# peterdavidfagan/mujoco_robot_environments

Hardware: AMD Instinct MI355X
Metric: env steps/sec (whole node), RearrangementEnv batch=4096 at 1/2/4/8 MI355X (higher is better)
Workload: dtype f32

## Files before the change

mujoco_robot_environments_amd/csrc/mre_api.cpp:

```cpp
#include <hip/hip_runtime.h>

#include <cmath>
#include <cstdio>
#include <cstdlib>
#include <cstring>
#include <string>
#include <algorithm>
#include <vector>

#include "mre_env.h"
#include "mre_labels.h"
#include "mre_heightmap.h"
#include "mre_warp.h"
#include "mre_launch.h"
#include "mre_model.h"
#include "mre_records.h"

using namespace mre;

static thread_local std::string g_err;
int mre::fail(int code, const std::string& msg) {
  g_err = msg;
  return code;
}

extern "C" const char* mre_last_error(void) { return g_err.c_str(); }

static int create_buffers(mre_env* e, int num_envs, int device_id) {
  e->N = num_envs;
  e->device = device_id;
  HIPCHK(hipSetDevice(device_id));
  HIPCHK(hipStreamCreateWithFlags(&e->stream, hipStreamNonBlocking));
  const size_t N = (size_t)num_envs;
  HIPCHK(hipMalloc(&e->dM, sizeof(DevModel)));
  HIPCHK(hipMemcpy(e->dM, &e->hM, sizeof(DevModel), hipMemcpyHostToDevice));
  HIPCHK(hipMalloc(&e->qpos, N * NQP * 4)); HIPCHK(hipMalloc(&e->qvel, N * NVP * 4));
  HIPCHK(hipMalloc(&e->qacc_ws, N * NVP * 4)); HIPCHK(hipMalloc(&e->ctrl, N * NU * 4));
  HIPCHK(hipMalloc(&e->qfine, N * QFINE_ROW * 4)); HIPCHK(hipMalloc(&e->sv_qfine, N * QFINE_ROW * 4));
  HIPCHK(hipMemsetAsync(e->qfine, 0, N * QFINE_ROW * 4, e->stream));
  HIPCHK(hipMalloc(&e->nstep, N * 4)); HIPCHK(hipMalloc(&e->sv_nstep, N * 4));
  HIPCHK(hipMemsetAsync(e->nstep, 0, N * 4, e->stream));
  HIPCHK(hipMalloc(&e->nprops, N * 4)); HIPCHK(hipMalloc(&e->prop_size, N * NPROP * 3 * 4));
  HIPCHK(hipMalloc(&e->osc_target, N * 16 * 4)); HIPCHK(hipMalloc(&e->grip_closed, N));
  HIPCHK(hipMalloc(&e->converged, N)); HIPCHK(hipMalloc(&e->mask, N));
  HIPCHK(hipMalloc(&e->sites, N * 16 * 4));
  HIPCHK(hipMalloc(&e->status, N * 4)); HIPCHK(hipMalloc(&e->stats, N * 4 * 4));
  HIPCHK(hipMalloc(&e->order, N * 4)); HIPCHK(hipMalloc(&e->auto_order, N * 4));
  HIPCHK(hipHostMalloc((void**)&e->h_auto_order, N * 4, hipHostMallocDefault));
  HIPCHK(hipStreamCreateWithFlags(&e->stream2, hipStreamNonBlocking));
  HIPCHK(hipEventCreateWithFlags(&e->ev_fork, hipEventDisableTiming));
  HIPCHK(hipEventCreateWithFlags(&e->ev_join, hipEventDisableTiming));
  HIPCHK(hipMalloc(&e->d_large, N)); HIPCHK(hipMalloc(&e->mask_r, N));
  HIPCHK(hipMalloc(&e->sv_qpos, N * NQP * 4)); HIPCHK(hipMalloc(&e->sv_qvel, N * NVP * 4));
  HIPCHK(hipMalloc(&e->sv_qacc_ws, N * NVP * 4)); HIPCHK(hipMalloc(&e->sv_ctrl, N * NU * 4));
  HIPCHK(hipMalloc(&e->sv_status, N * 4));
  HIPCHK(hipMalloc(&e->sv_converged, N));
  HIPCHK(hipHostMalloc((void**)&e->h_launch_info, mre_env::RING * N * 16, hipHostMallocMapped | hipHostMallocCoherent));
  HIPCHK(hipHostGetDevicePointer((void**)&e->d_launch_info, e->h_launch_info, 0));
  memset(e->h_launch_info, 0xFF, mre_env::RING * N * 16);
  HIPCHK(hipHostMalloc((void**)&e->h_info_last, N * 16, hipHostMallocDefault));
  memset(e->h_info_last, 0xFF, N * 16);
  HIPCHK(hipHostMalloc((void**)&e->h_large_stage, mre_env::NSTAGE * N, hipHostMallocMapped | hipHostMallocCoherent));
  HIPCHK(hipHostGetDevicePointer((void**)&e->d_large_stage, e->h_large_stage, 0));
  memset(e->h_large_stage, 0, mre_env::NSTAGE * N);
  HIPCHK(hipMalloc(&e->d_pending, N));
  HIPCHK(hipMemsetAsync(e->d_pending, 0, N, e->stream));
  HIPCHK(hipMemsetAsync(e->d_large, 0, N, e->stream));
  e->h_large.assign(N, 0); e->h_rerun.assign(N, 0);
  { int rc = sched_create(e); if (rc) return rc; }
  if (const char* fb = getenv("MRE_NO_FALLBACK")) e->fallback = atoi(fb) == 0;
  if (const char* ng = getenv("MRE_NARROW_GENERIC")) e->base_flags = atoi(ng) != 0 ? F_CLIP_ALWAYS : 0u;
  if (const char* fl = getenv("MRE_FORCE_LARGE")) {
    if (atoi(fl) != 0) {
      e->h_large.assign(N, 1); e->n_large = num_envs;
      HIPCHK(hipMemsetAsync(e->d_large, 1, N, e->stream));
    }
  }
  HIPCHK(hipMemsetAsync(e->status, 0, N * 4, e->stream)); HIPCHK(hipMemsetAsync(e->stats, 0, N * 16, e->stream));
  HIPCHK(hipMemsetAsync(e->grip_closed, 0, N, e->stream)); HIPCHK(hipMemsetAsync(e->osc_target, 0, N * 64, e->stream));
  HIPCHK(hipMemsetAsync(e->sites, 0, N * 64, e->stream));
  std::vector<int> np(N, NPROP);
  std::vector<float> ps(N * NPROP * 3, 0.0155f);
  HIPCHK(hipMemcpy(e->nprops, np.data(), N * 4, hipMemcpyHostToDevice));
  HIPCHK(hipMemcpy(e->prop_size, ps.data(), ps.size() * 4, hipMemcpyHostToDevice));
  e->osc = OscConfig{350.f, 20.f, 500.f, 100.f, 200.f, 30.f, {0.f, -0.785f, 0.f, -2.356f, 0.f, 1.571f, 0.785f},
                     5e-3f, 68e-3f, 0};
  HIPCHK(hipMalloc(&e->d_osc, sizeof(OscConfig)));
  HIPCHK(hipMemcpy(e->d_osc, &e->osc, sizeof(OscConfig), hipMemcpyHostToDevice));
  HIPCHK(hipStreamSynchronize(e->stream));
  int rc = mre_reset(e, nullptr);
  if (rc != MRE_OK) return rc;
  return mre_sync(e);
}

extern "C" int mre_create(const void* blob, size_t nbytes, int num_envs, int device_id, mre_env** out) {
  if (!blob || !out || num_envs <= 0) return fail(MRE_ERR_ARG, "mre_create: bad argument");
  *out = nullptr;
  mre_env* e = new mre_env();
  const std::string err = build_model(blob, nbytes, e->hM, e->solver);
  if (!err.empty()) { delete e; return fail(MRE_ERR_MODEL, err); }
  if (const char* it = getenv("MRE_DEBUG_ITERS")) e->hM.opt_rec.iterations = atoi(it);
  int rc;
  int ndev = 0;
  if (hipGetDeviceCount(&ndev) != hipSuccess || ndev <= 0) {
    delete e;
    return fail(MRE_ERR_NOGPU, "mre_create: no HIP device visible (the HIP path has no CPU fallback)");
  }
  if (device_id < 0 || device_id >= ndev) {
    delete e;
    return fail(MRE_ERR_ARG, "mre_create: device_id out of range");
  }
  rc = create_buffers(e, num_envs, device_id);
  if (rc != MRE_OK) {
    const std::string msg = g_err;
    mre_destroy(e);
    g_err = msg;
    return rc;
  }
  *out = e;
  return MRE_OK;
}

extern "C" int mre_destroy(mre_env* e) {
  if (!e) return MRE_OK;
  (void)hipSetDevice(e->device);
  (void)drain(e);
  if (getenv("MRE_DEBUG_TIMING") && e->dbg_calls > 0)
    fprintf(stderr, "mre: %ld pipelined calls, %.1f us per call in the library, of which %.1f us waiting for launch info\n",
            e->dbg_calls, 1e6 * e->dbg_call_s / e->dbg_calls, 1e6 * e->dbg_wait_s / e->dbg_calls);
  sched_destroy(e);
  for (float* p : e->seq_copy) if (p) (void)hipFree(p);
  if (e->stream) (void)hipStreamSynchronize(e->stream);
  if (e->stream2) (void)hipStreamSynchronize(e->stream2);
  void* ptrs[] = {e->dM, e->qpos, e->qvel, e->qacc_ws, e->ctrl, e->nprops, e->prop_size, e->osc_target,
                  e->grip_closed, e->converged, e->mask, e->sites, e->status, e->stats, e->d_osc, e->d_osc_env, e->order,
                  e->geoms, e->prop_rgb, e->bg_depth, e->bg_rgb, e->bg_seg,
                  e->d_large, e->mask_r, e->qfine, e->sv_qfine, e->nstep, e->sv_nstep, e->sv_qpos, e->sv_qvel, e->sv_qacc_ws, e->sv_ctrl,
                  e->sv_status, e->auto_order, e->sv_converged, e->contacts, e->contacts_full, e->settle_steps,
                  e->d_env_ids, e->ps_attempts, e->ps_prop, e->ps_tick, e->ps_which, e->ps_bounds, e->ps_pose, e->ps_zones,
                  e->ps_pick};
  for (void* p : ptrs) if (p) (void)hipFree(p);
  if (e->h_launch_info) (void)hipHostFree(e->h_launch_info);
  if (e->h_info_last) (void)hipHostFree(e->h_info_last);
  if (e->h_large_stage) (void)hipHostFree(e->h_large_stage);
  if (e->d_pending) (void)hipFree(e->d_pending);
  if (e->h_auto_order) (void)hipHostFree(e->h_auto_order);
  for (auto& pr : e->events) { (void)hipEventDestroy(pr.first); (void)hipEventDestroy(pr.second); }
  if (e->ev_order) (void)hipEventDestroy(e->ev_order);
  if (e->ev_fork) (void)hipEventDestroy(e->ev_fork);
  if (e->ev_join) (void)hipEventDestroy(e->ev_join);
  if (e->stream2) (void)hipStreamDestroy(e->stream2);
  if (e->stream) (void)hipStreamDestroy(e->stream);
  delete e;
  return MRE_OK;
}

extern "C" int mre_num_envs(const mre_env* e) { return e ? e->N : 0; }
extern "C" void* mre_stream(mre_env* e) { return e ? (void*)e->stream : nullptr; }
extern "C" int mre_sync(mre_env* e) {
  if (!e) return fail(MRE_ERR_ARG, "null handle");
  HIPCHK(hipSetDevice(e->device));
  DRAIN(e);
  HIPCHK(hipStreamSynchronize(e->stream));
  return MRE_OK;
}

static int copy_in(mre_env* e, void* dst, const void* src, size_t n) {
  HIPCHK(hipSetDevice(e->device));
  HIPCHK(hipMemcpyAsync(dst, src, n, hipMemcpyDefault, e->stream));
  return MRE_OK;
}
static int copy_out(mre_env* e, void* dst, const void* src, size_t n) {
  HIPCHK(hipSetDevice(e->device));
  HIPCHK(hipMemcpyAsync(dst, src, n, hipMemcpyDefault, e->stream));
  HIPCHK(hipStreamSynchronize(e->stream));
  return MRE_OK;
}
static int stage_mask(mre_env* e, const uint8_t* mask, const uint8_t** dmask) {
  *dmask = nullptr;
  if (!mask) return MRE_OK;
  int rc = copy_in(e, e->mask, mask, (size_t)e->N);
  *dmask = e->mask;
  return rc;
}

extern "C" int mre_set_props(mre_env* e, const int32_t* nprops, const float* prop_half_size) {
  if (!e || !nprops || !prop_half_size) return fail(MRE_ERR_ARG, "mre_set_props: null");
  DRAIN(e);
  int rc = copy_in(e, e->nprops, nprops, (size_t)e->N * 4);
  if (rc) return rc;
  return copy_in(e, e->prop_size, prop_half_size, (size_t)e->N * NPROP * 3 * 4);
}

extern "C" int mre_reset(mre_env* e, const uint8_t* mask) {
  if (!e) return fail(MRE_ERR_ARG, "null handle");
  DRAIN(e);
  HIPCHK(hipSetDevice(e->device));
  const uint8_t* dmask;
  int rc = stage_mask(e, mask, &dmask);
  if (rc) return rc;
  mre_launch_reset(e->dM, e->N, e->qpos, e->qvel, e->qacc_ws, e->qfine, e->ctrl, e->status, e->nstep, dmask, e->stream);
  HIPCHK(hipGetLastError());
  if (!mask) e->tick_tail_valid = false;
  bool changed = false;
  std::vector<uint8_t> hmask;
  if (mask) {
    hmask.resize((size_t)e->N);
    rc = copy_out(e, hmask.data(), dmask, (size_t)e->N);
    if (rc) return rc;
  }
  for (int i = 0; i < e->N; i++)
    if (!e->large_only && e->h_large[i] && (!mask || hmask[i])) { e->h_large[i] = 0; e->n_large--; changed = true; }
  if (changed) {
    HIPCHK(hipMemcpyAsync(e->d_large, e->h_large.data(), (size_t)e->N, hipMemcpyHostToDevice, e->stream));
    HIPCHK(hipStreamSynchronize(e->stream));
  }
  return MRE_OK;
}

static void fill_args(mre_env* e, StepArgs& a);
static bool is_device_ptr(const void* p) {
  hipPointerAttribute_t at;
  if (hipPointerGetAttributes(&at, p) != hipSuccess) { (void)hipGetLastError(); return false; }
  return at.type == hipMemoryTypeDevice;
// ... 1127 lines not shown
```

mujoco_robot_environments_amd/csrc/mre_dev.h:

```cpp
#pragma once
#include <stdint.h>

namespace mre {

constexpr int NB = 20;
constexpr int NRB = 16;
constexpr int GRIP_BODY0 = 8;
constexpr int NV = 39;
constexpr int NRV = 15;
constexpr int NQ = 43;
constexpr int NQP = 44;
constexpr int TRACE_W = 88;
constexpr int TRACE_QVEL = 48;
constexpr int NVP = 40;
constexpr int NU = 8;
constexpr int QFINE = 32;
constexpr int QFINE_ROW = 96;
constexpr int QFINE_CUBE_Q = 32;
constexpr int QFINE_CUBE_V = 60;
static_assert(QFINE_CUBE_Q + 7 * 4 == QFINE_CUBE_V && QFINE_CUBE_V + 6 * 4 <= QFINE_ROW, "qfine row layout");
constexpr int NPROP = 4;
constexpr int NG = 20;
constexpr int PROP_GEOM0 = 12;
constexpr int NPAIR = 128;
constexpr int NMR = 96;
constexpr int NSITE = 2;
constexpr int NEQ = 3;
constexpr int CONTACT_EXPORT = 32;
constexpr int MAXCHAIN = 9;
constexpr int ROBOT_DOF_PARENT[NRV] = {-1, 0, 1, 2, 3, 4, 5, 6, 7, 6, 9, 6, 11, 6, 13};
constexpr int robot_dof_depth(int i) { return ROBOT_DOF_PARENT[i] < 0 ? 0 : 1 + robot_dof_depth(ROBOT_DOF_PARENT[i]); }
constexpr int robot_dof_madr(int i) { return i == 0 ? 0 : robot_dof_madr(i - 1) + robot_dof_depth(i - 1) + 1; }
constexpr int robot_dof_anc(int i, int k) {
  int j = ROBOT_DOF_PARENT[i];
  for (int t = 0; t < k && j >= 0; t++) j = ROBOT_DOF_PARENT[j];
  return j;
}
static_assert(robot_dof_madr(NRV) == NMR, "robot mass-matrix size");

#if defined(MRE_LARGE_CAPS) && defined(MRE_NEWTON)
constexpr int NCON_MAX = 48;
constexpr int NEFC_MAX = 160;
constexpr int NRROW_MAX = 100;
constexpr int NPP_MAX = 16;
constexpr int MAXBLK = 58;
#elif defined(MRE_LARGE_CAPS)
constexpr int NCON_MAX = 44;
constexpr int NEFC_MAX = 148;
constexpr int NRROW_MAX = 83;
constexpr int NPP_MAX = 16;
constexpr int MAXBLK = 52;
#elif defined(MRE_NEWTON)
constexpr int NCON_MAX = 32;
constexpr int NEFC_MAX = 112;
constexpr int NRROW_MAX = 69;
constexpr int NPP_MAX = 8;
constexpr int MAXBLK = 40;
#else
constexpr int NCON_MAX = 32;
constexpr int NEFC_MAX = 112;
constexpr int NRROW_MAX = 62;
constexpr int NPP_MAX = 8;
constexpr int MAXBLK = 40;
#endif
constexpr int NRROW_MAX_COMPACT_PGS = 62, NRROW_MAX_COMPACT_NEWTON = 69;
#if !defined(MRE_LARGE_CAPS)
static_assert(NRROW_MAX ==
#ifdef MRE_NEWTON
              NRROW_MAX_COMPACT_NEWTON,
#else
              NRROW_MAX_COMPACT_PGS,
#endif
              "host-side copy of the compact robot-row capacity");
#endif
static_assert(NEFC_MAX <= 256 && NRROW_MAX < 127 && NPP_MAX <= 16 && MAXBLK >= 8 + NCON_MAX,
              "capacities must fit the block descriptor fields (mre_solver.h)");

struct alignas(16) PairRec {
  int g1, g2, b1, b2;
  int pid1, pid2, type1, single;
  float pos1[3], rb1;
  float pos2[3], rb2;
  float quat1[4], quat2[4];
  float size1[3], margin;
  float size2[3], gap;
};
static_assert(sizeof(PairRec) == 128, "PairRec is eight 16-byte words");

struct alignas(16) BodyRec {
  float quat[4];
  float pos[3], mass;
  float jnt_pos[3], qpos0;
  float jnt_axis[3]; int qposadr;
  float ipos[3]; int propid;
  float iquat[4];
  float inertia[3]; int dofadr;
  float jnt_range[2], invweight0[2];
  float jnt_stiffness, jnt_springref; int parent, jnt_limited;
};
static_assert(sizeof(BodyRec) == 144, "BodyRec is nine 16-byte words");
struct alignas(16) DofRec {
  int body, propid, dofadr, ten;
  float armature, damping, invweight0, ten_coef;
  float jnt_stiffness, jnt_springref, act_gain, act_bias0;
  float act_bias1, act_bias2, act_ctrl_lo, act_ctrl_hi;
  float act_force_lo, act_force_hi; int act_forcelimited, pad;
};
static_assert(sizeof(DofRec) == 80, "DofRec is five 16-byte words");
struct alignas(16) MEntryRec {
  int i, j; float armature, damping;
  float act_bias2, ten_coef; int ten, pad;
};
static_assert(sizeof(MEntryRec) == 32, "MEntryRec is two 16-byte words");
struct alignas(16) RowRec {
  float solref[2], margin, gap;
  float solimp[5], friction;
  float invw1, invw2;
};
static_assert(sizeof(RowRec) == 48, "RowRec is three 16-byte words");
constexpr int ROWREC_JNT = NEQ, ROWREC_PAIR = NEQ + NB, NROWREC = NEQ + NB + NPAIR;
struct alignas(16) EqRec {
  int type, b1, b2, pb1;
  int pb2, root, pad0, pad1;
  float data[8];
  float qpos0_1, qpos0_2; int pad2, root_chain_len;
  int root_chain[12];
};
static_assert(sizeof(EqRec) == 128 && MAXCHAIN <= 12, "EqRec is eight 16-byte words");
struct alignas(16) SiteRec {
  float pos[3]; int body;
  float quat[4];
};
static_assert(sizeof(SiteRec) == 32, "SiteRec is two 16-byte words");
struct alignas(16) OptRec {
  float timestep, impratio, tolerance; int iterations;
  float gravity[3]; int cone;
  float ten_coef[2]; int ten_dof[2];
  float grip_gainprm, grip_biasprm[3];
  float grip_forcerange[2], grip_ctrlrange[2];
  float robot_mass, M0_diag_robot_sum; int tcp_site, eef_site;
  float tcp_pos[3]; int pad;
};
static_assert(sizeof(OptRec) == 112, "OptRec is seven 16-byte words");

struct DevModel {
  int body_propid[NB];
  int chain_len[NB];
  int chain_dof[NB][MAXCHAIN];
  float body_mass[NB];
  int dof_Madr[NV + 1];
  float qpos0[NQP];
  int M_i[NMR], M_j[NMR];
  int geom_type[NG], geom_body[NG], geom_propid[NG];
  float geom_size[NG][3], geom_pos[NG][3], geom_quat[NG][4], geom_rbound[NG];
  int pair_g1[NPAIR], pair_g2[NPAIR];
  float pair_margin[NPAIR];
  PairRec pair_rec[NPAIR];
  float act_ctrlrange[NU][2];
  float home_qpos[7];
  float park_pos[NPROP][3];
  BodyRec body_rec[NB];
  DofRec dof_rec[NV];
  MEntryRec m_rec[NMR];
  RowRec row_rec[NROWREC];
  EqRec eq_rec[NEQ];
  SiteRec site_rec[NSITE];
  OptRec opt_rec;
};

struct OscConfig {
  float kp_pos, kd_pos, kp_ori, kd_ori, kp_null, kd_null;
  float null_q[7];
  float pos_thresh, ori_thresh;
  int pinv_always;
};

enum StepFlags : unsigned { F_NO_CONSTRAINTS = 1u, F_FREEZE_ROBOT = 2u, F_CONV_CONTINUE = 4u, F_CONV_OPEN = 8u,
                            F_OSC_EVAL = 16u, F_DETECT = 32u, F_SETTLE_EXIT = 64u, F_DETECT_ACTIVE = 128u,
                            F_CLIP_ALWAYS = 256u };
enum CtrlMode : int { CTRL_HELD = 0, CTRL_SEQ = 1, CTRL_OSC = 2 };

struct StepArgs {
  const DevModel* M;
  int N;
  float* qpos;
  float* qvel;
  float* qacc_ws;
  float* qfine;
  float* ctrl;
  const float* ctrl_seq;
  int seq_stride;
  const int* nprops;
  const float* prop_size;
  int nsteps, control_steps, mode;
  unsigned flags;
  const OscConfig* osc;
  int osc_stride;
  const float* osc_target;
  const uint8_t* grip_closed;
  uint8_t* converged;
  float* sites;
  uint32_t* status;
  int* nstep;
  int* stats;
  float* trace;
  int trace_nenv, trace_max, trace_base;
  const uint8_t* env_mask;
  const int* env_order;
  float* geoms;
  float* contacts;
  float* contacts_full;
  int* settle_steps;
  int min_settle_steps;
  const uint8_t* large;
  int want_large;
  float *sv_qpos, *sv_qvel, *sv_qacc_ws, *sv_qfine, *sv_ctrl;
  int* sv_nstep;
  uint32_t* sv_status;
  uint8_t* sv_converged;
  int* launch_info;
  uint8_t* pending;
  int* q_head;
  int* q_tail;
  int* q_buf;
  int* q_acc;
  int* q_done;
  int* q_started;
  const int* q_gen;
  int q_gen_expect;
  int q_wait;
  int* q_err;
  int q_nticks, q_shards, q_cap, q_stride;
  int q_lshards, q_capl;
};
constexpr int QUEUE_TICKS_MAX = 256;
constexpr int QUEUE_SHARDS_MAX = 32;
constexpr int QUEUE_LSHARDS_MAX = 16;

struct SearchArgs {
  const DevModel* M;
  int N;
  float* qpos;
  const int* nprops;
  const float* prop_size;
  const uint8_t* env_mask;
  const long long* env_ids;
  long long env_id_offset;
  unsigned long long seed;
  const int* prop;
  int fixed_prop;
  const double* bounds;
  double shared_bounds[6];
  const int* tick_base;
  long long tick0;
  int max_attempts;
  int yaw_mode;
  double fixed_quat[4];
  float max_dist;
  int commit;
  float* qfine;
  double* pose;
  int* attempts;
  unsigned flags;
};

constexpr int DYN_W = 128;
constexpr int DYN_JAC = 0, DYN_MASS = 42, DYN_BIAS = 91, DYN_POS = 98, DYN_QUAT = 101, DYN_QPOS = 105, DYN_QVEL = 112,
              DYN_PAD = 119;
struct DynArgs {
  const DevModel* M;
  int N;
  const float* qpos;
  const float* qvel;
  const float* qfine;
  const int* nprops;
  const float* prop_size;
  int site;
  float* out;
};

struct SortArgs {
  const DevModel* M;
  int N;
  const float* qpos;
  const int* nprops;
  const double* zones;
  double place_z;
  int* which;
  double* pick;
  double* bounds;
};

struct RenderArgs {
  int N, height, width;
  const float* geoms;
  const int* nprops;
  const uint8_t* prop_rgb;
  float geom_rgb[NG][3];
  float cam_pos[3], cam_mat[9];
  float fy;
  float light_pos[3];
  float ambient, head_diffuse, light_diffuse;
  float checker[2][3], checker_size;
  float zfar;
  uint8_t* rgb;
  float* depth;
  uint8_t* seg;
  const uint8_t* env_mask;
  int g0, g1;
  const float* bg_depth;
  const uint8_t* bg_rgb;
  const uint8_t* bg_seg;
};

}
```

mujoco_robot_environments_amd/csrc/mre_kernels.hip:

```cpp
#include <hip/hip_runtime.h>

#include "mre_dev.h"
#include "mre_math.h"
#include "mre_collide.h"

namespace mre {
using ModelP = MRE_MODEL_PTR(DevModel);
#if defined(MRE_PHASE_STAMPS) && MRE_PHASE_STAMPS >= 4
__shared__ unsigned long long dbg_acc[4];
#endif

struct OscSm {
  float J[6][7], M[7][7], MiJt[7][6], Li[6][6], Lam[6][6], V[6][6], Jbar[7][6];
  float ep[3], eo[3], F[6], LF[6], tn[7], Jbt[6], xd[6], w[6];
};

struct alignas(8) Blk {
  uint16_t row0;
  uint8_t type, nrows;
  uint8_t rslot;
  uint8_t pa, pb;
  uint8_t primary : 4;
  uint8_t bslot : 4;
};

constexpr int TAB_BYTES = 8 * (MAXBLK * 5 + 1) + 4 * 48;
constexpr int FRAME_BYTES = (int)sizeof(OscSm) > 4 * (NB * 16) ? (int)sizeof(OscSm) : 4 * (NB * 16);
constexpr int R1_MIN = TAB_BYTES - FRAME_BYTES > 0 ? TAB_BYTES - FRAME_BYTES : 4;
constexpr int MD_LD = 17;

struct Sm {
  float qpos[NQP], qvel[NVP], qlo[QFINE], ctrl[NU];
  float qfrc_smooth[NVP], qacc_smooth[NVP], qacc[NVP], qfrc_bias[NVP], qfrc_con[NVP];
  union {
    struct { float xpos[NB][3], xquat[NB][4], xmat[NB][9]; };
    OscSm osc;
#ifdef MRE_NEWTON
    struct { float nw_Ma[NVP], nw_grad[NVP], nw_search[NVP], nw_Mv[NVP]; };
#endif
  };
#ifndef MRE_NEWTON
  char tab_room[R1_MIN];
#endif
  float cdof[NRV][6];
  union {
    struct { float con_pos[NCON_MAX][3], con_frame[NCON_MAX][9], con_dist[NCON_MAX]; };
#ifdef MRE_NEWTON
    struct { float jar[NEFC_MAX], frc[NEFC_MAX], jv[NEFC_MAX]; };
#else
    struct { float jar[NEFC_MAX], frc[NEFC_MAX], pyr_f[4 * NCON_MAX]; };
#endif
  };
  float com_robot[3];
  float site_xpos[NSITE][3], site_xmat[1][9];
#ifdef MRE_NEWTON
  float qM[NMR];
#else
  float qM[NMR], qLD[NMR], qLDinv[NRV + 1];
#endif
  float prop_mass[NPROP], prop_inertia[NPROP][3], prop_size[NPROP][3];
  union { float scratch[64]; int iscr[64]; };
  float osc_tgt[16];
  int nprops;
  int ncon, nefc, nl, nrrow, npp, overflow, solver_iters;
  int finger_contact;
  uint8_t con_pair[NCON_MAX], con_rslot[NCON_MAX], con_bslot[NCON_MAX], con_b1[NCON_MAX], con_b2[NCON_MAX];
  uint16_t lim_info[NRV + 1];
  union {
    float JpA[3 * NCON_MAX][6];
    struct {
      float cinert[NB][10], crb[NRB][10], gP[NRB - GRIP_BODY0][6], gC[NRB - GRIP_BODY0][6];
      double gpose[NRB - GRIP_BODY0][7];
    };
  };
  float JpB[3 * NPP_MAX][6];
  union {
    float Jr[NRROW_MAX][NRV];
    struct {
      float cdof_dot[NV][6], cvel[NB][6], cfrc[NB][6];
      alignas(8) double gI[NRB - GRIP_BODY0][10];
      double gS[NRB - GRIP_BODY0][6];
    };
  };
#ifdef MRE_NEWTON
  float efc_R[NEFC_MAX], efc_aref[NEFC_MAX];
  float frc_r[NRROW_MAX];
  float con_fric[NCON_MAX];
  float hc[NCON_MAX][6];
  float Md[NRV][MD_LD];
  alignas(8) float W[NV * (NV + 1) / 2];
  uint8_t rstate[NEFC_MAX];
  uint8_t clist[NPROP][NCON_MAX];
  uint8_t ccount[NPROP], cpl_robot, cpl_cubes;
  alignas(8) uint16_t jdesc[NEFC_MAX][4];
  float zrow[24];
#else
  float Br[NRROW_MAX][NRV];
  alignas(16) float blkrec[MAXBLK][16];
  Blk blk[MAXBLK];
  uint8_t sched[MAXBLK][8];
#endif
  uint16_t hdr[NEFC_MAX];

  int nblk, nsched;
};

#if defined(MRE_LARGE_CAPS)
static_assert(sizeof(Sm) <= 27136, "large-capacity Sm must fit 6 workgroups per CU");
#else
static_assert(sizeof(Sm) <= 20480, "compact Sm must fit 8 workgroups per CU");
#endif

#ifdef MRE_NEWTON
MRE_DEV float* mh_store(Sm& s) { return &s.JpA[0][0]; }
static_assert(sizeof(((Sm*)0)->JpA) >= sizeof(float) * NMR, "M - h dF/dv fits the head of the constraint block");
#else
MRE_DEV float* mh_store(Sm& s) { return s.qLD; }
#endif

struct BodyRegs {
  float anchor[3], axis[3], xipos[3], ximat[9];
};

MRE_DEV double robot_q(const Sm& s, int d) { return (double)s.qpos[d] + (double)s.qlo[d]; }
MRE_DEV double robot_v(const Sm& s, int d) { return (double)s.qvel[d] + (double)s.qlo[QFINE / 2 + d]; }

MRE_DEV bool prop_is_active(const Sm& s, int propid) { return propid < 0 || propid < s.nprops; }

struct BodyK {
  float quat[4], pos[3], mass, jnt_pos[3], qpos0, jnt_axis[3], ipos[3], iquat[4], inertia[3];
  int qposadr, propid, dofadr, parent;
};
MRE_DEV BodyK load_body(ModelP M, int b) {
  const auto* R = &M->body_rec[b];
  BodyK B;
#pragma unroll
  for (int k = 0; k < 4; k++) { B.quat[k] = R->quat[k]; B.iquat[k] = R->iquat[k]; }
#pragma unroll
  for (int k = 0; k < 3; k++) { B.pos[k] = R->pos[k]; B.jnt_pos[k] = R->jnt_pos[k]; B.jnt_axis[k] = R->jnt_axis[k];
                                B.ipos[k] = R->ipos[k]; B.inertia[k] = R->inertia[k]; }
  B.mass = R->mass; B.qpos0 = R->qpos0; B.qposadr = R->qposadr; B.propid = R->propid; B.dofadr = R->dofadr;
  B.parent = R->parent;
  return B;
}

MRE_DEV bool body_is_active(ModelP M, const Sm& s, int b) {
  int p = M->body_propid[b];
  return p < 0 || p < s.nprops;
}

MRE_DEV void sincos_poly_d(double x, double& sn, double& cs) {
  const double z = x * x;
  double ps = -1.0 / 1307674368000.0;
  ps = ps * z + 1.0 / 6227020800.0;
  ps = ps * z - 1.0 / 39916800.0;
  ps = ps * z + 1.0 / 362880.0;
// ... 1143 lines not shown
  if (QUEUE && !Q_LARGE && l == 0) __hip_atomic_fetch_add(a.q_started, 1, __ATOMIC_RELAXED, __HIP_MEMORY_SCOPE_AGENT);
  if (QUEUE && Q_LARGE && a.q_wait != 0) {
    for (unsigned idle = 0; q_load(a.q_gen) != a.q_gen_expect; ++idle) {
      if (idle > 1024u) return;
      __builtin_amdgcn_s_sleep(127);
    }
  }
 for (;;) {
  if (QUEUE) {
    if (!queue_pop(a, l, (int)(blockIdx.x % (unsigned)(Q_LARGE ? a.q_lshards : a.q_shards)), env, qtick, qshard)) return;
    if (qtick > 0 || Q_LARGE) __builtin_amdgcn_fence(__ATOMIC_ACQUIRE, "agent");
  }
  const int step_lo = QUEUE ? qtick * a.control_steps : 0, step_hi = QUEUE ? step_lo + a.control_steps : a.nsteps;
  if (QUEUE && !Q_LARGE && qtick == 0 && a.large != nullptr && a.large[env] != 0) continue;
  if (!QUEUE || (!Q_LARGE && qtick == 0)) {
#define MRE_PASS_SKIP { if (QUEUE) { if (l == 0) __hip_atomic_fetch_add(a.q_done, 1, __ATOMIC_RELAXED, __HIP_MEMORY_SCOPE_AGENT); continue; } return; }
  if (!QUEUE && a.large != nullptr && (a.large[env] != 0) != (a.want_large != 0)) return;
  if (a.env_mask != nullptr && a.env_mask[env] == 0) {
    if (a.launch_info != nullptr && l < 4) a.launch_info[(size_t)env * 4 + l] = -1;
    MRE_PASS_SKIP;
  }
  if (a.pending != nullptr && a.pending[env] != 0) {
    if (a.launch_info != nullptr && l < 4) a.launch_info[(size_t)env * 4 + l] = l == 0 ? -2 : -1;
    MRE_PASS_SKIP;
  }
#undef MRE_PASS_SKIP
  }
  ModelP M = (ModelP)a.M;

  const bool save = a.sv_qpos != nullptr && step_lo == 0;
  if (l < NQP) {
    const float v = a.qpos[(size_t)env * NQP + l];
    s.qpos[l] = v;
    if (save) a.sv_qpos[(size_t)env * NQP + l] = v;
  }
  if (l < NVP) {
    const float v = a.qvel[(size_t)env * NVP + l], w = a.qacc_ws[(size_t)env * NVP + l];
    s.qvel[l] = v;
    s.qacc[l] = w;
    s.qfrc_con[l] = 0.f;
    if (save) { a.sv_qvel[(size_t)env * NVP + l] = v; a.sv_qacc_ws[(size_t)env * NVP + l] = w; }
  }
  if (l < QFINE) {
    const float v = a.qfine != nullptr ? a.qfine[(size_t)env * QFINE_ROW + l] : 0.f;
    s.qlo[l] = v;
    if (save && a.qfine != nullptr) a.sv_qfine[(size_t)env * QFINE_ROW + l] = v;
  }
  if (save && a.qfine != nullptr && l < QFINE_ROW - QFINE)
    a.sv_qfine[(size_t)env * QFINE_ROW + QFINE + l] = a.qfine[(size_t)env * QFINE_ROW + QFINE + l];
  float cube_lo_keep = 0.f;
  if (QUEUE && !Q_LARGE && a.qfine != nullptr && l < QFINE_ROW - QFINE) cube_lo_keep = a.qfine[(size_t)env * QFINE_ROW + QFINE + l];
  if (l < NU) {
    const float v = a.ctrl[(size_t)env * NU + l];
    s.ctrl[l] = v;
    if (save) a.sv_ctrl[(size_t)env * NU + l] = v;
  }
  if (save && l == 0) {
    if (a.nstep != nullptr) a.sv_nstep[env] = a.nstep[env];
    a.sv_status[env] = a.status[env];
    a.sv_converged[env] = a.converged != nullptr ? a.converged[env] : (uint8_t)0;
  }
  if (l == 0) { s.nprops = a.nprops[env]; s.overflow = 0; s.ncon = 0; s.nefc = 0; s.solver_iters = 0; }
#ifdef MRE_NEWTON
  if (l < 24) s.zrow[l] = 0.f;
#endif
  if (l < NPROP * 3) {
    const float sz = a.prop_size[(size_t)env * NPROP * 3 + l];
    s.prop_size[l / 3][l % 3] = sz;
  }
  MRE_SYNC();
  if (l < NPROP) {
    const float m = M->body_mass[NRB + l];
    const float* z = s.prop_size[l];
    s.prop_mass[l] = m;
    s.prop_inertia[l][0] = m / 3.f * (z[1] * z[1] + z[2] * z[2]);
    s.prop_inertia[l][1] = m / 3.f * (z[0] * z[0] + z[2] * z[2]);
    s.prop_inertia[l][2] = m / 3.f * (z[0] * z[0] + z[1] * z[1]);
  }
  MRE_SYNC();

#if defined(MRE_PHASE_STAMPS) && MRE_PHASE_STAMPS >= 4
  if (l < 4) dbg_acc[l] = 0ull;
#endif
#ifdef MRE_PHASE_STAMPS
  unsigned long long stamp_acc[4] = {0, 0, 0, 0};
  unsigned long long stamp_t = __builtin_amdgcn_s_memtime();
#endif
  bool arm_converged = ((a.flags & F_CONV_CONTINUE) != 0 || (QUEUE && qtick > 0)) && a.converged != nullptr && a.converged[env] != 0;
  float grip_cmd = 0.f;
  const OscConfig* oscp = a.osc + (size_t)env * a.osc_stride;
  int hw_ncon = 0, hw_nefc = 0, hw_nrrow = 0, hw_npp = 0;
  const unsigned long long launch_t0 = __builtin_amdgcn_s_memtime();
  if (a.mode == CTRL_OSC) {
    if (l < 16) s.osc_tgt[l] = a.osc_target[(size_t)env * 16 + l];
    grip_cmd = a.grip_closed[env] ? M->act_ctrlrange[NU - 1][1] : M->act_ctrlrange[NU - 1][0];
    MRE_SYNC();
  }
  int steps_done = 0;
  bool settled = false;
  for (int step = step_lo; step < step_hi; ++step) {
    MRE_STAMP(7);
    position_stage(M, s, l);
    MRE_STAMP(12);
    MRE_STAMP(13);
    gripper_local(M, s, l);
    if ((a.flags & F_NO_CONSTRAINTS) == 0) connect_rows_local(M, s, l);
    MRE_STAMP(14);
    crb_mass_matrix(M, s, l);
    MRE_SYNC();
#ifndef MRE_NEWTON
    factor_robot_regs(s.qM, s.qLD, s.qLDinv);
#endif
    MRE_STAMP(15);
    MRE_STAMP(0);

    velocity_stage(M, s, l);
    MRE_SYNC();
    finger_bias(M, s, l);
    MRE_STAMP(1);
    const bool constrained = (a.flags & F_NO_CONSTRAINTS) == 0;
    if (constrained) {

      collide(M, s, l, false, (a.flags & F_CLIP_ALWAYS) != 0);
      MRE_STAMP(2);
      assemble_constraints(M, s, l);
#ifdef MRE_NEWTON
      nw_build_lists(s, l);
#else
      solve_robot_rows(s, l);
      assemble_blocks(M, s, l);
#endif
      MRE_STAMP(3);
      hw_ncon = max(hw_ncon, s.ncon); hw_nefc = max(hw_nefc, s.nefc);
      hw_nrrow = max(hw_nrrow, s.nrrow); hw_npp = max(hw_npp, s.npp);
    }

    if (a.mode == CTRL_SEQ && (step % a.control_steps) == 0) {
      const int tick = step / a.control_steps;
      if (l < NU) s.ctrl[l] = a.ctrl_seq[((size_t)tick * a.seq_stride + env) * NU + l];
      MRE_SYNC();
    }
    if (a.mode == CTRL_OSC && (step % a.control_steps) == 0) {
      if (step > 0 && osc_converged(M, s, oscp, s.osc_tgt)) arm_converged = true;
      osc_compute(M, s, osc, oscp, s.osc_tgt, l);
      if (l == 0) s.ctrl[NU - 1] = grip_cmd;
      MRE_SYNC();
    }
    MRE_STAMP(4);
    const unsigned clamped = smooth_forces(M, s, l);
    MRE_STAMP(5);
    bool polished = false;
    if (constrained) {
#if defined(MRE_NEWTON) && defined(MRE_PHASE_STAMPS)
      newton_solve(M, s, l, stamp_acc, stamp_t);
      polished = nw_robot_polish(M, s, l);
#elif defined(MRE_NEWTON)
      newton_solve(M, s, l);
      polished = nw_robot_polish(M, s, l);
#else
      if (M->opt_rec.cone == 0) solve_constraints_pyramidal(M, s, l);
      else solve_constraints(M, s, l);
#endif
      MRE_STAMP(6);
    } else {
      if (l < NVP) { s.qacc[l] = s.qacc_smooth[l]; s.qfrc_con[l] = 0.f; }
      MRE_SYNC();
    }

    integrate_setup(M, s, l, clamped);
    factor_solve_robot(mh_store(s), s.scratch, l);
    integrate(M, s, l, a.flags, polished, a.qfine != nullptr ? a.qfine + (size_t)env * QFINE_ROW + QFINE_CUBE_Q : nullptr);
    steps_done = step + 1 - step_lo;
    if ((a.flags & F_SETTLE_EXIT) != 0) {
      float mv = 0.f, ma = 0.f;
      if (l >= NRV && l < NRV + 6 * s.nprops) { mv = fabsf(s.qvel[l]); ma = fabsf(s.qacc[l]); }
      mv = wave_max(mv); ma = wave_max(ma);
      settled = mv < 1e-3f && ma < 1e-2f && step + 1 > a.min_settle_steps;
    }
    if (a.trace != nullptr && env < a.trace_nenv && (a.trace_base + step) < a.trace_max) {
      if (l < TRACE_QVEL) {
        float v = l < NQ ? s.qpos[l] : 0.f;
        if (l == NQ && constrained) {
          int mask = 0;
          for (int k = 0; k < s.nl; k++) mask |= 1 << ((s.lim_info[k] & 0xFF) - 1);
          v = (float)(s.ncon + 64 * mask);
        }
        if (l == NQ + 1 && constrained) {
          unsigned h = 0u;
          for (int c = 0; c < s.ncon; c++) {
            const int pr = s.con_pair[c];
            const unsigned key = (unsigned)(M->pair_g1[pr] * 32 + M->pair_g2[pr] + 1);
            h = (h + key * key) & 0x3FFFFFu;
          }
          v = (float)h;
        }
        if (l == NQ + 2 && constrained && M->opt_rec.cone != 0) {
          unsigned h = 0u;
          const int ns = 7 + s.nl;
          for (int i = 7; i < ns; i++) h += (s.frc[i] > 0.f ? 1u : 2u) * (unsigned)((i + 1) * (i + 1));
          for (int c = 0; c < s.ncon; c++) {
            const int i = ns + 3 * c;
#ifdef MRE_NEWTON
            const float mu = s.con_fric[c];
#else
            const float mu = s.blkrec[8 + c][15];
#endif
            const float fn = s.frc[i], ft2 = s.frc[i + 1] * s.frc[i + 1] + s.frc[i + 2] * s.frc[i + 2], lim = mu * fn;
            const unsigned z = fn <= 0.f ? 1u : (ft2 >= lim * lim * (1.f - 1e-4f) ? 3u : 2u);
            h += z * (unsigned)((c + 3) * (c + 3));
          }
          v = (float)(h & 0x3FFFFFu);
        }
        a.trace[((size_t)(a.trace_base + step) * a.trace_nenv + env) * TRACE_W + l] = v;
      }
      if (l < NVP) a.trace[((size_t)(a.trace_base + step) * a.trace_nenv + env) * TRACE_W + TRACE_QVEL + l] = l < NV ? s.qvel[l] : 0.f;
    }
    if (settled) break;
  }
  MRE_STAMP(7);
  if (a.settle_steps != nullptr && l == 0) a.settle_steps[env] = settled ? steps_done : -steps_done;
  const bool hand_over = QUEUE && !Q_LARGE && s.overflow != 0;
  if (a.nstep != nullptr && l == 0 && !hand_over) {
    if (QUEUE) __hip_atomic_fetch_add(a.nstep + env, steps_done, __ATOMIC_RELAXED, __HIP_MEMORY_SCOPE_AGENT);
    else a.nstep[env] += steps_done;
  }
  if (a.nsteps == 0 && (a.flags & F_OSC_EVAL) != 0 && a.mode == CTRL_OSC) {
    position_stage(M, s, l);
    gripper_local(M, s, l);
    crb_mass_matrix(M, s, l);
    MRE_SYNC();
    velocity_stage(M, s, l);
    MRE_SYNC();
    osc_compute(M, s, osc, oscp, s.osc_tgt, l);
    if (l == 0) s.ctrl[NU - 1] = grip_cmd;
    MRE_SYNC();
  }
  if (a.nsteps == 0 && (a.flags & F_DETECT) != 0 && a.contacts != nullptr) {
    position_stage(M, s, l);
    collide(M, s, l, (a.flags & F_DETECT_ACTIVE) == 0, (a.flags & F_CLIP_ALWAYS) != 0);
    float* o = a.contacts + (size_t)env * (1 + 3 * CONTACT_EXPORT);
    const int n = s.ncon < CONTACT_EXPORT ? s.ncon : CONTACT_EXPORT;
    if (l == 0) o[0] = s.overflow ? -(float)s.ncon : (float)s.ncon;
    if (l < n) {
      const int pr = s.con_pair[l];
      o[1 + 3 * l] = (float)M->pair_g1[pr]; o[2 + 3 * l] = (float)M->pair_g2[pr]; o[3 + 3 * l] = s.con_dist[l];
      if (a.contacts_full != nullptr) {
        float* f = a.contacts_full + ((size_t)env * CONTACT_EXPORT + l) * 12;
        for (int k = 0; k < 3; k++) f[k] = s.con_pos[l][k];
        for (int k = 0; k < 9; k++) f[3 + k] = s.con_frame[l][k];
      }
    }
    MRE_SYNC();
    if (l == 0) s.overflow = 0;
  }
  const bool q_last = !QUEUE || (qtick + 1 == a.q_nticks && !hand_over);
  if (q_last && (a.mode == CTRL_OSC || a.sites != nullptr || a.geoms != nullptr)) kinematics_only(M, s, l);
  if (a.mode == CTRL_OSC && a.nsteps > 0 && !hand_over) {
    if (q_last && osc_converged(M, s, oscp, s.osc_tgt)) arm_converged = true;
    if (l == 0) {
      if (a.converged != nullptr) a.converged[env] = arm_converged ? 1 : 0;
      if (q_last && !arm_converged && a.status != nullptr && (a.flags & F_CONV_OPEN) == 0) {
        if (QUEUE) __hip_atomic_fetch_or(a.status + env, 1u, __ATOMIC_RELAXED, __HIP_MEMORY_SCOPE_AGENT);
        else a.status[env] |= 1u;
      }
    }
  }
  if (a.geoms != nullptr && l < NG) {
    float p[3], R[9], size[3], rb;
    geom_pose(M, s, l, p, R, size, &rb);
    float* o = a.geoms + ((size_t)env * NG + l) * 16;
    const int pid = M->geom_propid[l];
    const bool active = pid < 0 || pid < s.nprops;
    for (int k = 0; k < 3; k++) o[k] = p[k];
    for (int k = 0; k < 9; k++) o[3 + k] = R[k];
    for (int k = 0; k < 3; k++) o[12 + k] = size[k];
    o[15] = active ? (float)M->geom_type[l] : -1.f;
  }
  if (a.sites != nullptr && q_last) {
    float* o = a.sites + (size_t)env * 16;
    if (l < 3) o[l] = s.site_xpos[M->opt_rec.tcp_site][l];
    if (l >= 3 && l < 6) o[l] = s.site_xpos[M->opt_rec.eef_site][l - 3];
    if (l == 6) {
      float q[4];
      mat2q(q, s.site_xmat[0]);
      o[6] = q[0]; o[7] = q[1]; o[8] = q[2]; o[9] = q[3];
    }
  }
  if (hand_over) {
    if (a.qfine != nullptr && l < QFINE_ROW - QFINE) a.qfine[(size_t)env * QFINE_ROW + QFINE + l] = cube_lo_keep;
  } else {
    if (l < NQP) a.qpos[(size_t)env * NQP + l] = s.qpos[l];
    if (l < NVP) {
      a.qvel[(size_t)env * NVP + l] = s.qvel[l];
      a.qacc_ws[(size_t)env * NVP + l] = l < NV ? s.qacc[l] : 0.f;
    }
    if (l < QFINE && a.qfine != nullptr) a.qfine[(size_t)env * QFINE_ROW + l] = s.qlo[l];
    if (l < NU) a.ctrl[(size_t)env * NU + l] = s.ctrl[l];
  }
  const bool q_more = QUEUE && !hand_over && qtick + 1 < a.q_nticks;
  if (l == 0 && a.launch_info != nullptr) {
    int* li = a.launch_info + (size_t)env * 4;
    unsigned long long dt = (__builtin_amdgcn_s_memtime() - launch_t0) >> 10;
    int moved = 0;
    if (QUEUE) {
      int* qa = a.q_acc + (size_t)env * 4;
      if (qtick > 0 || Q_LARGE) {
        hw_ncon = max(hw_ncon, q_load(qa + 0) & 0xFFFF); hw_nefc = max(hw_nefc, q_load(qa + 1));
        hw_nrrow = max(hw_nrrow, q_load(qa + 2) & 0xFFFF); hw_npp = max(hw_npp, q_load(qa + 2) >> 16);
        dt += (unsigned long long)q_load(qa + 3);
        moved = q_load(qa + 0) >> 16;
// ... 437 lines not shown
```

mujoco_robot_environments_amd/csrc/mre_model.cpp:

```cpp
#include "mre_model.h"

#include <cstdint>
#include <cstring>
#include <vector>

#include "../../include/mre.h"

namespace mre {

namespace {
struct Blob {
  const unsigned char* p;
  size_t n;
  bool find(const char* name, uint32_t* code, uint32_t* count, uint64_t* off) const {
    uint32_t ne;
    memcpy(&ne, p + 8, 4);
    const unsigned char* t = p + 16;
    for (uint32_t k = 0; k < ne; k++, t += 48)
      if (strncmp((const char*)t, name, 32) == 0) {
        memcpy(code, t + 32, 4); memcpy(count, t + 36, 4); memcpy(off, t + 40, 8);
        return *off + (size_t)(*count) * (*code ? 8 : 4) <= n;
      }
    return false;
  }
  bool ints(const char* name, int* dst, int expect) const {
    uint32_t c, cnt; uint64_t off;
    if (!find(name, &c, &cnt, &off) || c != 0 || (int)cnt != expect) return false;
    memcpy(dst, p + off, 4 * (size_t)cnt);
    return true;
  }
  bool flts(const char* name, float* dst, int expect) const {
    uint32_t c, cnt; uint64_t off;
    if (!find(name, &c, &cnt, &off) || c != 1 || (int)cnt != expect) return false;
    for (uint32_t k = 0; k < cnt; k++) {
      double v;
      memcpy(&v, p + off + 8 * (size_t)k, 8);
      dst[k] = (float)v;
    }
    return true;
  }
};
}

#define RI(name, dst, n) if (!b.ints(name, (int*)(dst), n)) return std::string("model entry ") + name
#define RF(name, dst, n) if (!b.flts(name, (float*)(dst), n)) return std::string("model entry ") + name

static bool same_bits(const void* a, const void* b, size_t n) { return memcmp(a, b, n) == 0; }
static std::string pack_records(const ModelTables& t, DevModel& m) {
  if (t.ten_dof[0] == t.ten_dof[1] || t.ten_dof[0] < 0 || t.ten_dof[0] >= NRV || t.ten_dof[1] < 0 || t.ten_dof[1] >= NRV)
    return "the gripper tendon must couple two different robot dofs";
  for (int e = 0; e < NEQ; e++)
    for (int k = 0; k < 2; k++)
      if (t.eq_obj[e][k] < 1 || t.eq_obj[e][k] >= NRB) return "equality constraints must couple robot bodies";
  if (t.tcp_site < 0 || t.tcp_site >= NSITE || t.eef_site < 0 || t.eef_site >= NSITE) return "tcp_site / eef_site name no site";
  for (int b = 1; b < NRB; b++)
    if (t.body_parent[b] != ROBOT_DOF_PARENT[b - 1] + 1) return "robot body tree differs from the one the kernels are unrolled for (mre_dev.h)";
  for (int d = 0; d < NV; d++)
    if (t.dof_body[d] != (d < NRV ? d + 1 : NRB + (d - NRV) / 6)) return "dof layout differs from the compiled kernels";
  auto ten_of = [&](int d) { return d == t.ten_dof[0] ? 0 : (d == t.ten_dof[1] ? 1 : -1); };
  for (int b = 0; b < NB; b++) {
    BodyRec& r = m.body_rec[b];
    memset(&r, 0, sizeof(r));
    for (int c = 0; c < 4; c++) { r.quat[c] = t.body_quat[b][c]; r.iquat[c] = t.body_iquat[b][c]; }
    for (int c = 0; c < 3; c++) { r.pos[c] = t.body_pos[b][c]; r.ipos[c] = t.body_ipos[b][c]; r.jnt_pos[c] = t.jnt_pos[b][c];
                                  r.jnt_axis[c] = t.jnt_axis[b][c]; r.inertia[c] = t.body_inertia[b][c]; }
    for (int c = 0; c < 2; c++) { r.jnt_range[c] = t.jnt_range[b][c]; r.invweight0[c] = t.body_invweight0[b][c]; }
    r.mass = t.body_mass[b]; r.qposadr = t.body_qposadr[b]; r.dofadr = t.body_dofadr[b]; r.propid = t.body_propid[b];
    r.qpos0 = (r.qposadr >= 0 && r.qposadr < NQ) ? t.qpos0[r.qposadr] : 0.f;
    r.jnt_stiffness = t.jnt_stiffness[b]; r.jnt_springref = t.jnt_springref[b];
    r.parent = t.body_parent[b]; r.jnt_limited = t.jnt_limited[b];
  }
  for (int d = 0; d < NV; d++) {
    DofRec& r = m.dof_rec[d];
    memset(&r, 0, sizeof(r));
    const int b = t.dof_body[d];
    if (b < 0 || b >= NB) return "dof_bodyid names a body that does not exist";
    r.body = b; r.propid = t.body_propid[b]; r.dofadr = t.body_dofadr[b]; r.ten = ten_of(d);
    r.armature = t.dof_armature[d]; r.damping = t.dof_damping[d]; r.invweight0 = t.dof_invweight0[d];
    r.ten_coef = r.ten >= 0 ? t.ten_coef[r.ten] : 0.f;
    r.jnt_stiffness = t.jnt_stiffness[b]; r.jnt_springref = t.jnt_springref[b];
    if (d < 7) {
      r.act_gain = t.act_gain[d]; r.act_bias0 = t.act_bias[d][0]; r.act_bias1 = t.act_bias[d][1]; r.act_bias2 = t.act_bias[d][2];
      r.act_ctrl_lo = t.act_ctrlrange[d][0]; r.act_ctrl_hi = t.act_ctrlrange[d][1];
      r.act_force_lo = t.act_forcerange[d][0]; r.act_force_hi = t.act_forcerange[d][1];
      r.act_forcelimited = t.act_forcelimited[d];
    }
  }
  for (int e = 0; e < NMR; e++) {
    MEntryRec& r = m.m_rec[e];
    memset(&r, 0, sizeof(r));
    r.i = t.M_i[e]; r.j = t.M_j[e];
    r.armature = t.dof_armature[r.i]; r.damping = t.dof_damping[r.i];
    r.act_bias2 = r.i < 7 ? t.act_bias[r.i][2] : 0.f;
    r.ten = ten_of(r.i); r.ten_coef = r.ten >= 0 ? t.ten_coef[r.ten] : 0.f;
  }
  for (int k = 0; k < NROWREC; k++) memset(&m.row_rec[k], 0, sizeof(RowRec));
  for (int e = 0; e < NEQ; e++) {
    RowRec& r = m.row_rec[e];
    const int b1 = t.eq_obj[e][0], b2 = t.eq_obj[e][1];
    for (int c = 0; c < 2; c++) r.solref[c] = t.eq_solref[e][c];
    for (int c = 0; c < 5; c++) r.solimp[c] = t.eq_solimp[e][c];
    r.invw1 = e < 2 ? t.body_invweight0[b1][0] : t.dof_invweight0[b1 - 1];
    r.invw2 = e < 2 ? t.body_invweight0[b2][0] : t.dof_invweight0[b2 - 1];
    EqRec& q = m.eq_rec[e];
    memset(&q, 0, sizeof(q));
    q.type = t.eq_type[e]; q.b1 = b1; q.b2 = b2; q.pb1 = t.body_parent[b1]; q.pb2 = t.body_parent[b2];
    q.root = b1;
    while (q.root >= GRIP_BODY0) q.root = t.body_parent[q.root];
    for (int c = 0; c < 8; c++) q.data[c] = t.eq_data[e][c];
    q.qpos0_1 = t.qpos0[b1 - 1]; q.qpos0_2 = t.qpos0[b2 - 1];
    q.root_chain_len = t.chain_len[q.root];
    for (int c = 0; c < MAXCHAIN; c++) q.root_chain[c] = t.chain_dof[q.root][c];
  }
  for (int b = 1; b < NRB; b++) {
    RowRec& r = m.row_rec[ROWREC_JNT + b];
    for (int c = 0; c < 2; c++) r.solref[c] = t.jnt_solref[b][c];
    for (int c = 0; c < 5; c++) r.solimp[c] = t.jnt_solimp[b][c];
    r.invw1 = t.dof_invweight0[b - 1];
  }
  for (int k = 0; k < NPAIR; k++) {
    if (t.pair_g1[k] < 0) continue;
    RowRec& r = m.row_rec[ROWREC_PAIR + k];
    const int b1 = t.geom_body[t.pair_g1[k]], b2 = t.geom_body[t.pair_g2[k]];
    for (int c = 0; c < 2; c++) r.solref[c] = t.pair_solref[k][c];
    for (int c = 0; c < 5; c++) r.solimp[c] = t.pair_solimp[k][c];
    r.margin = t.pair_margin[k]; r.gap = t.pair_gap[k]; r.friction = t.pair_friction[k][0];
    r.invw1 = (b1 > 0 && b1 < NRB) ? t.body_invweight0[b1][0] : 0.f;
    r.invw2 = (b2 > 0 && b2 < NRB) ? t.body_invweight0[b2][0] : 0.f;
  }
  for (int k = 0; k < NSITE; k++) {
    SiteRec& r = m.site_rec[k];
    memset(&r, 0, sizeof(r));
    if (t.site_body[k] < 0 || t.site_body[k] >= NB) return "site_bodyid names a body that does not exist";
    r.body = t.site_body[k];
    for (int c = 0; c < 3; c++) r.pos[c] = t.site_pos[k][c];
    for (int c = 0; c < 4; c++) r.quat[c] = t.site_quat[k][c];
  }
  {
    OptRec& o = m.opt_rec;
    memset(&o, 0, sizeof(o));
    o.timestep = t.timestep; o.impratio = t.impratio; o.tolerance = t.tolerance; o.iterations = t.iterations;
    for (int c = 0; c < 3; c++) { o.gravity[c] = t.gravity[c]; o.grip_biasprm[c] = t.grip_biasprm[c]; }
    o.cone = t.cone;
    for (int c = 0; c < 2; c++) { o.ten_coef[c] = t.ten_coef[c]; o.ten_dof[c] = t.ten_dof[c]; o.grip_forcerange[c] = t.grip_forcerange[c];
                                  o.grip_ctrlrange[c] = t.act_ctrlrange[NU - 1][c]; }
    o.grip_gainprm = t.grip_gainprm; o.robot_mass = t.robot_mass; o.M0_diag_robot_sum = t.M0_diag_robot_sum;
    o.tcp_site = t.tcp_site; o.eef_site = t.eef_site;
    for (int c = 0; c < 3; c++) o.tcp_pos[c] = t.site_pos[t.tcp_site][c];
  }

  bool ok = true;
#define SAME(a, b) ok = ok && sizeof(a) == sizeof(b) && same_bits(&(a), &(b), sizeof(a))
  for (int b = 0; b < NB && ok; b++) {
    const BodyRec& r = m.body_rec[b];
    SAME(r.quat, t.body_quat[b]); SAME(r.pos, t.body_pos[b]); SAME(r.mass, t.body_mass[b]); SAME(r.jnt_pos, t.jnt_pos[b]);
    SAME(r.jnt_axis, t.jnt_axis[b]); SAME(r.qposadr, t.body_qposadr[b]); SAME(r.ipos, t.body_ipos[b]);
    SAME(r.propid, t.body_propid[b]); SAME(r.iquat, t.body_iquat[b]); SAME(r.inertia, t.body_inertia[b]);
    SAME(r.dofadr, t.body_dofadr[b]); SAME(r.jnt_range, t.jnt_range[b]); SAME(r.invweight0, t.body_invweight0[b]);
    SAME(r.jnt_stiffness, t.jnt_stiffness[b]); SAME(r.jnt_springref, t.jnt_springref[b]); SAME(r.parent, t.body_parent[b]);
    SAME(r.jnt_limited, t.jnt_limited[b]);
    if (b >= 1) SAME(r.qpos0, t.qpos0[t.body_qposadr[b]]);
  }
  for (int d = 0; d < NV && ok; d++) {
    const DofRec& r = m.dof_rec[d];
    const int b = t.dof_body[d];
    SAME(r.body, t.dof_body[d]); SAME(r.propid, t.body_propid[b]); SAME(r.dofadr, t.body_dofadr[b]);
    ok = ok && r.ten == (d == t.ten_dof[0] ? 0 : (d == t.ten_dof[1] ? 1 : -1));
    SAME(r.armature, t.dof_armature[d]); SAME(r.damping, t.dof_damping[d]); SAME(r.invweight0, t.dof_invweight0[d]);
    if (r.ten >= 0) SAME(r.ten_coef, t.ten_coef[r.ten]);
    SAME(r.jnt_stiffness, t.jnt_stiffness[b]); SAME(r.jnt_springref, t.jnt_springref[b]);
    if (d < 7) {
      SAME(r.act_gain, t.act_gain[d]); SAME(r.act_bias0, t.act_bias[d][0]); SAME(r.act_bias1, t.act_bias[d][1]);
      SAME(r.act_bias2, t.act_bias[d][2]); SAME(r.act_ctrl_lo, t.act_ctrlrange[d][0]); SAME(r.act_ctrl_hi, t.act_ctrlrange[d][1]);
      SAME(r.act_force_lo, t.act_forcerange[d][0]); SAME(r.act_force_hi, t.act_forcerange[d][1]);
      SAME(r.act_forcelimited, t.act_forcelimited[d]);
    }
  }
  for (int e = 0; e < NMR && ok; e++) {
    const MEntryRec& r = m.m_rec[e];
    SAME(r.i, t.M_i[e]); SAME(r.j, t.M_j[e]);
    const int i = t.M_i[e];
    SAME(r.armature, t.dof_armature[i]); SAME(r.damping, t.dof_damping[i]);
    if (i < 7) SAME(r.act_bias2, t.act_bias[i][2]);
    ok = ok && r.ten == (i == t.ten_dof[0] ? 0 : (i == t.ten_dof[1] ? 1 : -1));
    if (r.ten >= 0) SAME(r.ten_coef, t.ten_coef[r.ten]);
  }
  for (int e = 0; e < NEQ && ok; e++) {
    const RowRec& r = m.row_rec[e];
    const EqRec& q = m.eq_rec[e];
    const int b1 = t.eq_obj[e][0], b2 = t.eq_obj[e][1];
    SAME(r.solref, t.eq_solref[e]); SAME(r.solimp, t.eq_solimp[e]);
    if (e < 2) { SAME(r.invw1, t.body_invweight0[b1][0]); SAME(r.invw2, t.body_invweight0[b2][0]); }
    else { SAME(r.invw1, t.dof_invweight0[b1 - 1]); SAME(r.invw2, t.dof_invweight0[b2 - 1]); }
    SAME(q.type, t.eq_type[e]); SAME(q.b1, t.eq_obj[e][0]); SAME(q.b2, t.eq_obj[e][1]);
    SAME(q.pb1, t.body_parent[b1]); SAME(q.pb2, t.body_parent[b2]); SAME(q.data, t.eq_data[e]);
    SAME(q.qpos0_1, t.qpos0[b1 - 1]); SAME(q.qpos0_2, t.qpos0[b2 - 1]);
    int root = b1;
    while (root >= GRIP_BODY0) root = t.body_parent[root];
    ok = ok && q.root == root;
    SAME(q.root_chain_len, t.chain_len[root]);
    for (int c = 0; c < MAXCHAIN; c++) SAME(q.root_chain[c], t.chain_dof[root][c]);
  }
  for (int b = 1; b < NRB && ok; b++) {
    const RowRec& r = m.row_rec[ROWREC_JNT + b];
    SAME(r.solref, t.jnt_solref[b]); SAME(r.solimp, t.jnt_solimp[b]); SAME(r.invw1, t.dof_invweight0[b - 1]);
  }
  for (int k = 0; k < NPAIR && ok; k++) {
    if (t.pair_g1[k] < 0) continue;
    const RowRec& r = m.row_rec[ROWREC_PAIR + k];
    const int b1 = t.geom_body[t.pair_g1[k]], b2 = t.geom_body[t.pair_g2[k]];
    SAME(r.solref, t.pair_solref[k]); SAME(r.solimp, t.pair_solimp[k]); SAME(r.margin, t.pair_margin[k]);
    SAME(r.gap, t.pair_gap[k]); SAME(r.friction, t.pair_friction[k][0]);
    if (b1 > 0 && b1 < NRB) SAME(r.invw1, t.body_invweight0[b1][0]);
    if (b2 > 0 && b2 < NRB) SAME(r.invw2, t.body_invweight0[b2][0]);
  }
  for (int k = 0; k < NSITE && ok; k++) {
    const SiteRec& r = m.site_rec[k];
    SAME(r.body, t.site_body[k]); SAME(r.pos, t.site_pos[k]); SAME(r.quat, t.site_quat[k]);
  }
  {
    const OptRec& o = m.opt_rec;
    SAME(o.timestep, t.timestep); SAME(o.impratio, t.impratio); SAME(o.tolerance, t.tolerance); SAME(o.iterations, t.iterations);
    SAME(o.gravity, t.gravity); SAME(o.cone, t.cone); SAME(o.ten_coef, t.ten_coef); SAME(o.ten_dof, t.ten_dof);
    SAME(o.grip_gainprm, t.grip_gainprm); SAME(o.grip_biasprm, t.grip_biasprm); SAME(o.grip_forcerange, t.grip_forcerange);
    SAME(o.grip_ctrlrange, t.act_ctrlrange[NU - 1]); SAME(o.robot_mass, t.robot_mass);
    SAME(o.M0_diag_robot_sum, t.M0_diag_robot_sum); SAME(o.tcp_site, t.tcp_site); SAME(o.eef_site, t.eef_site);
    SAME(o.tcp_pos, t.site_pos[t.tcp_site]);
  }
#undef SAME
  if (!ok) return "a packed model record differs from the table it was filled from";
  return std::string();
}

std::string build_model(const void* blob, size_t nbytes, DevModel& m, int& solver) {
  if (nbytes < 16) return "blob too small";
  Blob b{(const unsigned char*)blob, nbytes};
  uint32_t magic;
  memcpy(&magic, b.p, 4);
  if (magic != 0x4D524542u) return "bad blob magic";
  uint32_t nentry;
  memcpy(&nentry, b.p + 8, 4);
  if (16 + 48 * (size_t)nentry > nbytes) return "blob too small";
  ModelTables t;
  memset(&t, 0, sizeof(t));
  memset(&m, 0, sizeof(m));
  int nbody, nv, nq, nM, ngeom, nsite, npair, neq, nprop, nu;
  RI("nbody", &nbody, 1); RI("nv", &nv, 1); RI("nq", &nq, 1); RI("nM", &nM, 1); RI("ngeom", &ngeom, 1);
  RI("nsite", &nsite, 1); RI("npair", &npair, 1); RI("neq", &neq, 1); RI("nprop", &nprop, 1);
  RI("nu", &nu, 1);
  if (nbody != NB || nv != NV || nq != NQ || ngeom != NG || nsite != NSITE || npair > NPAIR ||
      neq != NEQ || nprop != NPROP || nu != NU)
    return "scene dimensions differ from the compiled kernels";
  int body_jnttype[NB], act_dof[NU];
  RI("body_parentid", t.body_parent, NB); RI("body_jnttype", body_jnttype, NB);
  RI("body_dofadr", t.body_dofadr, NB); RI("body_qposadr", t.body_qposadr, NB);
  RI("body_propid", t.body_propid, NB);
  RF("body_pos", t.body_pos, NB * 3); RF("body_quat", t.body_quat, NB * 4);
  RF("body_ipos", t.body_ipos, NB * 3); RF("body_iquat", t.body_iquat, NB * 4);
  RF("body_mass", t.body_mass, NB); RF("body_inertia", t.body_inertia, NB * 3);
  RF("body_invweight0", t.body_invweight0, NB * 2);
  RF("jnt_pos", t.jnt_pos, NB * 3); RF("jnt_axis", t.jnt_axis, NB * 3); RF("jnt_range", t.jnt_range, NB * 2);
  RF("jnt_stiffness", t.jnt_stiffness, NB); RF("jnt_springref", t.jnt_springref, NB);
  RF("jnt_solref", t.jnt_solref, NB * 2); RF("jnt_solimp", t.jnt_solimp, NB * 5);
  RI("jnt_limited", t.jnt_limited, NB);
  RI("dof_bodyid", t.dof_body, NV); RI("dof_parentid", t.dof_parent, NV); RI("dof_Madr", t.dof_Madr, NV);
  t.dof_Madr[NV] = nM;
  RF("dof_armature", t.dof_armature, NV); RF("dof_damping", t.dof_damping, NV);
  RF("dof_invweight0", t.dof_invweight0, NV); RF("qpos0", t.qpos0, NQ);
  RI("geom_type", t.geom_type, NG); RI("geom_bodyid", t.geom_body, NG); RI("geom_propid", t.geom_propid, NG);
  RF("geom_size", t.geom_size, NG * 3); RF("geom_pos", t.geom_pos, NG * 3);
  RF("geom_quat", t.geom_quat, NG * 4); RF("geom_rbound", t.geom_rbound, NG);
  {
    std::vector<int> pg(2 * npair);
    RI("pair_geom", pg.data(), 2 * npair);
    for (int k = 0; k < NPAIR; k++) { t.pair_g1[k] = -1; t.pair_g2[k] = -1; }
    for (int k = 0; k < npair; k++) { t.pair_g1[k] = pg[2 * k]; t.pair_g2[k] = pg[2 * k + 1]; }
  }
  RI("pair_single", t.pair_single, npair);
  RF("pair_friction", t.pair_friction, npair * 3); RF("pair_solref", t.pair_solref, npair * 2);
  RF("pair_solimp", t.pair_solimp, npair * 5); RF("pair_margin", t.pair_margin, npair);
  RF("pair_gap", t.pair_gap, npair);
  for (int k = 0; k < NPAIR; k++) {
    PairRec& r = m.pair_rec[k];
    memset(&r, 0, sizeof(r));
    r.g1 = t.pair_g1[k]; r.g2 = t.pair_g2[k];
    if (r.g1 < 0) { r.g2 = -1; r.b1 = r.b2 = 0; r.pid1 = r.pid2 = -1; continue; }
    if (r.g1 >= NG || r.g2 < 0 || r.g2 >= NG) return "pair table names a geom that does not exist";
    r.b1 = t.geom_body[r.g1]; r.b2 = t.geom_body[r.g2];
    r.pid1 = t.geom_propid[r.g1]; r.pid2 = t.geom_propid[r.g2];
    r.type1 = t.geom_type[r.g1]; r.single = (t.pair_single[k] & 0xFF) | (t.geom_type[r.g2] << 8);
    if (t.geom_type[r.g1] == 2 || (t.geom_type[r.g2] == 2 && t.geom_type[r.g1] != 1))
      return "cylinder pairs: only box (geom 1) - cylinder (geom 2) is implemented";
    for (int c = 0; c < 3; c++) { r.pos1[c] = t.geom_pos[r.g1][c]; r.pos2[c] = t.geom_pos[r.g2][c];
                                  r.size1[c] = t.geom_size[r.g1][c]; r.size2[c] = t.geom_size[r.g2][c]; }
    for (int c = 0; c < 4; c++) { r.quat1[c] = t.geom_quat[r.g1][c]; r.quat2[c] = t.geom_quat[r.g2][c]; }
    r.rb1 = t.geom_rbound[r.g1]; r.rb2 = t.geom_rbound[r.g2];
    r.margin = t.pair_margin[k]; r.gap = t.pair_gap[k];
  }
  RI("site_bodyid", t.site_body, NSITE); RF("site_pos", t.site_pos, NSITE * 3);
  RF("site_quat", t.site_quat, NSITE * 4);
  RI("eef_site", &t.eef_site, 1); RI("tcp_site", &t.tcp_site, 1);
  RI("eq_type", t.eq_type, NEQ); RI("eq_obj", t.eq_obj, NEQ * 2); RF("eq_data", t.eq_data, NEQ * 8);
  RF("eq_solref", t.eq_solref, NEQ * 2); RF("eq_solimp", t.eq_solimp, NEQ * 5);
  RI("ten_dof", t.ten_dof, 2); RF("ten_coef", t.ten_coef, 2);
  RI("act_dof", act_dof, NU); RF("act_ctrlrange", t.act_ctrlrange, NU * 2);
  RF("grip_gainprm", &t.grip_gainprm, 1); RF("grip_biasprm", t.grip_biasprm, 3);
  RF("grip_forcerange", t.grip_forcerange, 2);
  for (int a = 0; a < NU; a++) { t.act_gain[a] = 1.f; t.act_forcelimited[a] = 0; }
  { uint32_t c, cnt; uint64_t off;
    if (b.find("act_gainprm", &c, &cnt, &off)) {
      RF("act_gainprm", t.act_gain, NU); RF("act_biasprm", t.act_bias, NU * 3);
      RF("act_forcerange", t.act_forcerange, NU * 2); RI("act_forcelimited", t.act_forcelimited, NU);
    } }
  RF("opt_timestep", &t.timestep, 1); RF("opt_gravity", t.gravity, 3); RF("opt_impratio", &t.impratio, 1);
  RF("opt_tolerance", &t.tolerance, 1); RI("opt_iterations", &t.iterations, 1);
  solver = MRE_SOLVER_PGS;
  { uint32_t c, cnt; uint64_t off; if (b.find("opt_solver", &c, &cnt, &off)) RI("opt_solver", &solver, 1); }
  if (solver != MRE_SOLVER_PGS && solver != MRE_SOLVER_NEWTON) return "opt_solver must be 0 (PGS) or 2 (Newton)";
  { uint32_t c, cnt; uint64_t off; int cone = 1;
    if (b.find("opt_cone", &c, &cnt, &off)) RI("opt_cone", &cone, 1);
    if (cone != 0 && cone != 1) return "opt_cone must be 0 (pyramidal) or 1 (elliptic)";
    t.cone = cone; }
  RF("home_qpos", t.home_qpos, 7);
  float M0d[NV];
  RF("M0_diag", M0d, NV);

  for (int bb = 1; bb < NB; bb++) {
    bool ok = bb < NRB ? (body_jnttype[bb] == 1 && t.body_dofadr[bb] == bb - 1 && t.body_qposadr[bb] == bb - 1 &&
                          t.body_propid[bb] < 0 && t.body_parent[bb] < bb)
                       : (body_jnttype[bb] == 2 && t.body_dofadr[bb] == NRV + 6 * (bb - NRB) &&
                          t.body_qposadr[bb] == NRV + 7 * (bb - NRB) && t.body_propid[bb] == bb - NRB &&
                          t.body_parent[bb] == 0);
    if (!ok) return "body layout differs from the compiled kernels";
  }
  if (t.dof_Madr[NRV] != NMR) return "robot mass-matrix size differs";
  for (int a = 0; a < 7; a++)
    if (act_dof[a] != a) return "arm actuators must drive dofs 0..6";

  int body_level[NB] = {0};
  for (int bb = 1; bb < NB; bb++) body_level[bb] = body_level[t.body_parent[bb]] + 1;
  for (int bb = 0; bb < NB; bb++)
    if (body_level[bb] > MAXCHAIN) return "tree deeper than MAXCHAIN";

  t.robot_mass = 0;
  for (int bb = 1; bb < NRB; bb++) {
    t.robot_mass += t.body_mass[bb];
    int chain[MAXCHAIN], n = 0;
    for (int d = t.body_dofadr[bb]; d >= 0; d = t.dof_parent[d]) {
      if (n >= MAXCHAIN) return "dof chain too long";
      chain[n++] = d;
    }
    t.chain_len[bb] = n;
    for (int k = 0; k < n; k++) t.chain_dof[bb][k] = chain[n - 1 - k];
  }
  for (int i = 0; i < NRV; i++) {
    int adr = t.dof_Madr[i];
    for (int j = i; j >= 0; j = t.dof_parent[j], adr++) { t.M_i[adr] = i; t.M_j[adr] = j; }
    if (adr != t.dof_Madr[i + 1]) return "dof_Madr inconsistent";
  }
  for (int i = 0; i < NRV; i++)
    if (t.dof_parent[i] != ROBOT_DOF_PARENT[i] || t.dof_Madr[i] != robot_dof_madr(i))
      return "robot dof tree differs from the one the kernels are unrolled for (mre_dev.h)";
  t.M0_diag_robot_sum = 0;
  for (int i = 0; i < NRV; i++) t.M0_diag_robot_sum += M0d[i];
  for (int p = 0; p < NPROP; p++) {
    t.park_pos[p][0] = 2.0f + 0.5f * p; t.park_pos[p][1] = 2.0f; t.park_pos[p][2] = -5.0f;
  }
#define KEEP(x) static_assert(sizeof(m.x) == sizeof(t.x), #x); memcpy(&m.x, &t.x, sizeof(m.x))
  KEEP(body_propid); KEEP(chain_len); KEEP(chain_dof); KEEP(body_mass);
  KEEP(dof_Madr); KEEP(qpos0); KEEP(M_i); KEEP(M_j);
  KEEP(geom_type); KEEP(geom_body); KEEP(geom_propid); KEEP(geom_size); KEEP(geom_pos); KEEP(geom_quat); KEEP(geom_rbound);
  KEEP(pair_g1); KEEP(pair_g2); KEEP(pair_margin);
  KEEP(act_ctrlrange); KEEP(home_qpos); KEEP(park_pos);
#undef KEEP
  std::string err = pack_records(t, m);
  if (!err.empty()) return err;
  int prop_geom0 = -1;
  for (int g = 0; g < NG; g++) if (t.geom_propid[g] == 0) prop_geom0 = g;
  if (prop_geom0 != PROP_GEOM0 || t.geom_type[1] != 1 || t.geom_body[1] != 0)
    return "mre_create: expected geom 1 = the table (static box) and one geom per cube slot";
  return std::string();
}

}
```

mujoco_robot_environments_amd/csrc/mre_newton.h:

```cpp
#pragma once

namespace mre {

constexpr int NW_QUAD = 0, NW_SAT = 1, NW_CONE = 4;
constexpr int NW_LS_MAX = 20;
constexpr float NW_LS_TOL = 0.01f;
#ifndef NW_LS_REL_VALUE
#define NW_LS_REL_VALUE 1e-5f
#endif
constexpr float NW_LS_REL = NW_LS_REL_VALUE;

MRE_DEV float rdlane(float v, int lane) {
  return __builtin_bit_cast(float, __builtin_amdgcn_readlane(__builtin_bit_cast(int, v), lane));
}
MRE_DEV int uni(int v) { return __builtin_amdgcn_readfirstlane(v); }
MRE_DEV float unif(float v) {
  return __builtin_bit_cast(float, __builtin_amdgcn_readfirstlane(__builtin_bit_cast(int, v)));
}

MRE_DEV float nw_Jl(const Sm& s, int i, int h, int l, int lp, int lk) {
  const int rs = h & 0xFF, pa = (h >> 8) & 0xF, pb = (h >> 12) & 0xF;
  float j = 0.f;
  if (l < NRV) {
    if (rs != HDR_NONE) j = s.Jr[rs][l];
// ... 162 lines not shown
#pragma unroll
      for (int q = 0; q < 8; q++)
        if (g0 + q < n) t[q] = rdlane(u, HI - g0 - q);
      __builtin_amdgcn_sched_barrier(0);
#pragma unroll
      for (int q = 0; q < 8; q++)
        if (g0 + q < n) hh[HI - g0 - q] = fmaf(-u, t[q], hh[HI - g0 - q]);
      __builtin_amdgcn_sched_barrier(0);
    }
  }
}

template <int K>
MRE_DEV void nw_elim_col(float (&hh)[NV], float& g, float& y, float& dinv, int l, unsigned nbm) {
  constexpr int blk = K < NRV ? 0 : 1 + (K - NRV) / 6;
  constexpr int b0 = blk == 0 ? 0 : NRV + 6 * (blk - 1);
  const float piv = rdlane(hh[K], K);
  const float d = __builtin_amdgcn_rsqf(fmaxf(piv, 1e-20f));
  const float u = hh[K] * d;
  hh[K] = u;
  const float yk = rdlane(g, K) * d;
  g = fmaf(-u, yk, g);
  y = (l == K) ? yk : y;
  dinv = (l == K) ? d : dinv;
  nw_elim_update<K - 1, b0>(hh, u);
  if constexpr (blk > 0) {
    if constexpr (blk > 3) { if (nbm & (1u << 3)) nw_elim_update<NRV + 17, NRV + 12>(hh, u); }
    if constexpr (blk > 2) { if (nbm & (1u << 2)) nw_elim_update<NRV + 11, NRV + 6>(hh, u); }
    if constexpr (blk > 1) { if (nbm & (1u << 1)) nw_elim_update<NRV + 5, NRV>(hh, u); }
    if (nbm & 1u) nw_elim_update<NRV - 1, 0>(hh, u);
  }
}
template <int K, int KEND>
MRE_DEV void nw_elim_range(float (&hh)[NV], float& g, float& y, float& dinv, int l, unsigned nbm) {
  nw_elim_col<K>(hh, g, y, dinv, l, nbm);
  if constexpr (K > KEND) nw_elim_range<K - 1, KEND>(hh, g, y, dinv, l, nbm);
}

struct NwPoint { float alpha, cost, d1, d2; };

MRE_PHASE_FN void nw_build_lists(Sm& s, int l) {
  const int kept = s.ncon;
  const bool on = l < kept;
  const int cb1 = on ? s.con_b1[l] : 0, cb2 = on ? s.con_b2[l] : 0;
  int pa = -1, pb = -1;
  if (cb1 >= NRB) pa = cb1 - NRB;
  if (cb2 >= NRB) { if (pa < 0) pa = cb2 - NRB; else pb = cb2 - NRB; }
  const unsigned long long lt = (1ull << l) - 1ull;
  const bool rob = on && pa >= 0 && s.con_rslot[on ? l : 0] != HDR_NONE;
  unsigned cr = 0u, cc = 0u;
#pragma unroll
  for (int p = 0; p < NPROP; p++) {
    const bool mine = on && (pa == p || pb == p);
    const unsigned long long m = __ballot(mine);
    if (mine) s.clist[p][__popcll(m & lt)] = (uint8_t)(pb == p ? (l | 0x80) : l);
    if (l == 0) s.ccount[p] = (uint8_t)__popcll(m);
    if (__ballot(rob && pa == p) != 0ull) cr |= 1u << p;
  }
  const int pairbit = (on && pb >= 0) ? cube_pair_bit(pa, pb) : -1;
#pragma unroll
  for (int b = 0; b < 6; b++)
    if (__ballot(pairbit == b) != 0ull) cc |= 1u << b;
  if (l == 0) { s.cpl_robot = (uint8_t)cr; s.cpl_cubes = (uint8_t)cc; }
  const int nscalar = 7 + s.nl;
  const unsigned zoff = (unsigned)offsetof(Sm, zrow);
  for (int i = l; i < s.nefc; i += 64) {
    const int h = s.hdr[i], ra = (h >> 8) & 0xF, rb = (h >> 12) & 0xF;
    const int crow = i - nscalar;
    const unsigned offA = crow >= 0 ? (unsigned)offsetof(Sm, JpA) + 24u * (unsigned)crow : zoff;
    const unsigned offB = (crow >= 0 && rb != 0xF)
                              ? (unsigned)offsetof(Sm, JpB) + 24u * (unsigned)(3 * s.con_bslot[crow / 3] + crow % 3) : zoff;
#pragma unroll
    for (int cb = 0; cb < NPROP; cb++) s.jdesc[i][cb] = (uint16_t)(ra == cb ? offA : (rb == cb ? offB : zoff));
  }
  MRE_SYNC();
}

struct NwLane {
  int lp, lk;
  bool lact;
  float mdiag;
  float mu_scale;
  float scale;
};
MRE_DEV NwLane nw_lane(ModelP M, const Sm& s, int l) {
  NwLane c;
  c.lp = (l >= NRV && l < NV) ? (l - NRV) / 6 : -1;
  c.lk = (l >= NRV && l < NV) ? (l - NRV) % 6 : 0;
  c.lact = l < NRV || (c.lp >= 0 && c.lp < s.nprops);
  c.mdiag = c.lp >= 0 ? (c.lk < 3 ? s.prop_mass[c.lp] : s.prop_inertia[c.lp][c.lk - 3]) : 0.f;
  c.mu_scale = __builtin_amdgcn_rsqf(fmaxf(M->opt_rec.impratio, kMinVal));
  float msum = M->opt_rec.M0_diag_robot_sum;
  for (int p = 0; p < s.nprops; p++)
    msum += 3.f * s.prop_mass[p] + s.prop_inertia[p][0] + s.prop_inertia[p][1] + s.prop_inertia[p][2];
  c.scale = 1.0f / msum;
  return c;
}

template <bool PYR>
MRE_DEV float nw_update_gradient(Sm& s, int l, const NwLane& c, int nscalar, int ncon) {
  const float sc = nw_update<true, PYR>(s, l, nscalar, ncon, c.mu_scale, s.jar);
  MRE_SYNC();
  const float qc = nw_JTf(s, l, c.lp, c.lk, nscalar);
  const bool on = l < NV && c.lact;
  const float fs = on ? s.qfrc_smooth[l] : 0.f, as = on ? s.qacc_smooth[l] : 0.f;
  const float qa = on ? s.qacc[l] : 0.f, Ma = on ? s.nw_Ma[l] : 0.f;
  if (l < NVP) {
    s.qfrc_con[l] = on ? qc : 0.f;
    s.nw_grad[l] = on ? Ma - fs - qc : 0.f;
  }
  const float cost = sc + wave_sum(0.5f * (Ma - fs) * (qa - as));
  MRE_SYNC();
  return cost;
}

template <bool PYR>
MRE_DEV float nw_setup_impl(ModelP M, Sm& s, int l) {
  const NwLane c = nw_lane(M, s, l);
  const int nefc = s.nefc, ncon = s.ncon, nscalar = 7 + s.nl;
  for (int e = l; e < NRV * MD_LD; e += 64) (&s.Md[0][0])[e] = 0.f;
  MRE_SYNC();
  for (int e = l; e < NMR; e += 64) {
    const int i = M->M_i[e], j = M->M_j[e];
    const float v = s.qM[e];
    s.Md[i][j] = v; s.Md[j][i] = v;
  }
  MRE_SYNC();
  const bool on = l < NV && c.lact;
  const float fs = on ? s.qfrc_smooth[l] : 0.f, as = on ? s.qacc_smooth[l] : 0.f;
  float qa = on ? s.qacc[l] : 0.f;
  float Ma = on ? nw_mulM(s, l, c.mdiag, s.qacc) : 0.f;
  for (int i = l; i < nefc; i += 64) {
    const float aref = s.efc_aref[i];
    float d1, d2;
    row_dot2(s, i, s.qacc, s.qacc_smooth, d1, d2);
    s.jar[i] = d1 - aref;
    s.jv[i] = d2 - aref;
  }
  MRE_SYNC();
  const float gauss = wave_sum(0.5f * (Ma - fs) * (qa - as));
  const float cost_ws = gauss + nw_update<false, PYR>(s, l, nscalar, ncon, c.mu_scale, s.jar);
  const float cost_sm = nw_update<false, PYR>(s, l, nscalar, ncon, c.mu_scale, s.jv);
  if (cost_ws > cost_sm || !(cost_ws == cost_ws)) {
    qa = as; Ma = fs;
    for (int i = l; i < nefc; i += 64) s.jar[i] = s.jv[i];
  }
  if (l < NVP) { s.qacc[l] = qa; s.nw_Ma[l] = Ma; }
  MRE_SYNC();
  return nw_update_gradient<PYR>(s, l, c, nscalar, ncon);
}
MRE_PHASE_FN float nw_setup(ModelP M, Sm& s, int l) { return nw_setup_impl<false>(M, s, l); }
MRE_PHASE_FN float nw_setup_pyramidal(ModelP M, Sm& s, int l) { return nw_setup_impl<true>(M, s, l); }

MRE_PHASE_FN void nw_direction(ModelP M, Sm& s, int l) {
  MRE_DBG_T0();
  const NwLane c = nw_lane(M, s, l);
  const int nefc = s.nefc, nscalar = 7 + s.nl, nprops = s.nprops;
  const int lp = c.lp, lk = c.lk;
  float hh[NV];
#pragma unroll
  for (int k = 0; k < NV; k++) {
    float v = 0.f;
    if (k < NRV) { if (l < NRV) v = s.Md[l][k]; }
    else if (l == k) v = c.lact ? c.mdiag : 1.0f;
    hh[k] = v;
  }
  MRE_DBG_STAMP(4, 0);
#if defined(MRE_PHASE_STAMPS) && MRE_PHASE_STAMPS == 5
  {
    int nc_ = 0, nq_ = 0;
    for (int r0 = 0; r0 < nefc; r0 += 64) {
      const int st_ = r0 + l < nefc ? (int)s.rstate[r0 + l] : NW_SAT;
      nc_ += __popcll(__ballot(st_ == NW_CONE)); nq_ += __popcll(__ballot(st_ == NW_QUAD));
    }
    if (threadIdx.x == 0) { dbg_acc[2] += (unsigned long long)nc_ << 4; dbg_acc[3] += (unsigned long long)nq_ << 4; }
  }
#endif
  typedef float v4f __attribute__((ext_vector_type(4)));
  v4f c00 = {0.f, 0.f, 0.f, 0.f}, c10 = c00, c11 = c00, c20 = c00, c21 = c00, c22 = c00;
  {
    const int g = l >> 4, m16 = l & 15;
    const char* const sb = reinterpret_cast<const char*>(&s);
    const unsigned zoff = (unsigned)offsetof(Sm, zrow), jr0 = (unsigned)offsetof(Sm, Jr);
    const unsigned sh = m16 < 12 ? 16u * (unsigned)(m16 / 6) : 0u;
    const unsigned lo = 4u * (unsigned)(m16 % 6), lr = 4u * (unsigned)m16;
    auto ldw = [&](unsigned off) { return *reinterpret_cast<const float*>(sb + off); };
    auto meta = [&](int r0, int& ii, int& st, int& h, float& R, uint2& d) {
      const int i = r0 + g;
      ii = i < nefc ? i : 0;
      st = i < nefc ? (int)s.rstate[ii] : NW_SAT;
      h = s.hdr[ii];
      R = s.efc_R[ii];
      d = *reinterpret_cast<const uint2*>(&s.jdesc[ii][0]);
    };
    auto gather = [&](int h, uint2 d, float& w0, float& w1, float& w2) {
      const int rs = h & 0xFF;
      w0 = ldw((rs != HDR_NONE ? jr0 + 60u * (unsigned)rs : zoff) + lr);
      w1 = ldw(((d.x >> sh) & 0xFFFFu) + lo);
      w2 = nprops > 2 ? ldw(((d.y >> sh) & 0xFFFFu) + lo) : 0.f;
    };
    static_assert(sizeof(s.Jr[0]) == 60 && sizeof(s.JpA[0]) == 24 && sizeof(s.JpB[0]) == 24, "row strides of the gathers");
    struct Meta { int ii, st, h; float R; uint2 d; };
    auto chunk = [&](const Meta& cur, Meta& nxt, int r0) {
      const int ii = cur.ii, h = cur.h, st = cur.st;
      const uint2 d = cur.d;
      const bool quad = st == NW_QUAD, cone = st == NW_CONE;
      const float D = quad ? __builtin_amdgcn_rcpf(cur.R) : 0.f;
      if (r0 + 4 < nefc) meta(r0 + 4, nxt.ii, nxt.st, nxt.h, nxt.R, nxt.d);
      float v0, v1, v2, a0, a1, a2;
      if (__any(cone)) {
        const int cr = ii - nscalar;
        const int k = cone ? cr % 3 : 0;
        const int i0 = ii - k, i1 = cone ? i0 + 1 : ii, i2 = cone ? i0 + 2 : ii;
        float x0, x1, x2, y0, y1, y2, z0, z1, z2;
        gather(s.hdr[i0], *reinterpret_cast<const uint2*>(&s.jdesc[i0][0]), x0, x1, x2);
        gather(s.hdr[i1], *reinterpret_cast<const uint2*>(&s.jdesc[i1][0]), y0, y1, y2);
        gather(s.hdr[i2], *reinterpret_cast<const uint2*>(&s.jdesc[i2][0]), z0, z1, z2);
        const float* hcp = s.hc[cone ? cr / 3 : 0];
        const float H0 = k == 0 ? hcp[0] : (k == 1 ? hcp[1] : hcp[2]);
        const float H1 = k == 0 ? hcp[1] : (k == 1 ? hcp[3] : hcp[4]);
        const float H2 = k == 0 ? hcp[2] : (k == 1 ? hcp[4] : hcp[5]);
        v0 = k == 0 ? x0 : (k == 1 ? y0 : z0);
        v1 = k == 0 ? x1 : (k == 1 ? y1 : z1);
        v2 = k == 0 ? x2 : (k == 1 ? y2 : z2);
        a0 = cone ? H0 * x0 + H1 * y0 + H2 * z0 : v0 * D;
        a1 = cone ? H0 * x1 + H1 * y1 + H2 * z1 : v1 * D;
        a2 = cone ? H0 * x2 + H1 * y2 + H2 * z2 : v2 * D;
      } else {
        gather(h, d, v0, v1, v2);
        a0 = v0 * D; a1 = v1 * D; a2 = v2 * D;
      }
      c00 = __builtin_amdgcn_mfma_f32_16x16x4f32(a0, v0, c00, 0, 0, 0);
      c10 = __builtin_amdgcn_mfma_f32_16x16x4f32(a1, v0, c10, 0, 0, 0);
      c11 = __builtin_amdgcn_mfma_f32_16x16x4f32(a1, v1, c11, 0, 0, 0);
      if (nprops > 2) {
        c20 = __builtin_amdgcn_mfma_f32_16x16x4f32(a2, v0, c20, 0, 0, 0);
        c21 = __builtin_amdgcn_mfma_f32_16x16x4f32(a2, v1, c21, 0, 0, 0);
        c22 = __builtin_amdgcn_mfma_f32_16x16x4f32(a2, v2, c22, 0, 0, 0);
      }
    };
    Meta mA, mB;
    meta(0, mA.ii, mA.st, mA.h, mA.R, mA.d);
    mB = mA;
    for (int r0 = 0; r0 < nefc; r0 += 8) {
      chunk(mA, mB, r0);
      if (r0 + 4 < nefc) chunk(mB, mA, r0 + 4);
    }
    MRE_DBG_STAMP(4, 1);
    float* T = s.W;
    constexpr int TS = 17;
    const int mytile = l < NRV ? 0 : (l < NRV + 12 ? 1 : (l < NV ? 2 : -1));
    const int mym = l < NRV ? l : (l < NRV + 12 ? l - NRV : l - NRV - 12);
    auto spill = [&](const v4f& cv, int off) {
#pragma unroll
      for (int v = 0; v < 4; v++) T[off + (4 * g + v) * TS + m16] = cv[v];
    };
#define NW_TILE(OFF, TI, TJ, BI, NI, BJ, NJ)                                                   \
    if (mytile == TI) {                                                                        \
      _Pragma("unroll") for (int n = 0; n < NJ; n++) hh[BJ + n] += T[OFF + mym * TS + n];      \
    }                                                                                          \
    if (TI != TJ && mytile == TJ) {                                                            \
      _Pragma("unroll") for (int q = 0; q < NI; q++) hh[BI + q] += T[OFF + q * TS + mym];      \
    }
    constexpr int T2 = 16 * TS;
    static_assert(2 * T2 <= NV * (NV + 1) / 2, "two tiles fit the factor's storage");
    spill(c00, 0); spill(c10, T2);
    MRE_SYNC();
    NW_TILE(0, 0, 0, 0, NRV, 0, NRV)
    if (nprops > 0) { NW_TILE(T2, 1, 0, NRV, 12, 0, NRV) }
    MRE_SYNC();
    if (nprops > 0) {
      spill(c11, 0); spill(c20, T2);
      MRE_SYNC();
      NW_TILE(0, 1, 1, NRV, 12, NRV, 12)
      if (nprops > 2) { NW_TILE(T2, 2, 0, NRV + 12, 12, 0, NRV) }
      MRE_SYNC();
    }
    if (nprops > 2) {
      spill(c21, 0); spill(c22, T2);
      MRE_SYNC();
      NW_TILE(0, 2, 1, NRV + 12, 12, NRV, 12)
      NW_TILE(T2, 2, 2, NRV + 12, 12, NRV + 12, 12)
      MRE_SYNC();
    }
#undef NW_TILE
  }
  MRE_DBG_STAMP(4, 2);
  unsigned adj[5];
  {
    const unsigned cr = s.cpl_robot, cq = s.cpl_cubes;
    adj[0] = 0u;
#pragma unroll
    for (int p = 0; p < NPROP; p++) {
      unsigned a = (cr >> p) & 1u;
#pragma unroll
      for (int q = 0; q < NPROP; q++)
        if (q != p && ((cq >> cube_pair_bit(p, q)) & 1u)) a |= 1u << (1 + q);
      adj[1 + p] = a;
    }
#pragma unroll
    for (int a = 4; a >= 1; a--) {
      const unsigned nb = adj[a] & ((1u << a) - 1u);
#pragma unroll
      for (int b = 1; b < 4; b++)
        if (b < a && ((nb >> b) & 1u)) adj[b] |= nb & ~(1u << b);
    }
#pragma unroll
    for (int a = 1; a < 5; a++) adj[a] = (unsigned)uni((int)adj[a]);
  }
  float g = l < NVP ? s.nw_grad[l] : 0.f, y = 0.f, dinv = 1.0f;
  if (nprops > 3) nw_elim_range<NRV + 23, NRV + 18>(hh, g, y, dinv, l, adj[4] & 0xFu);
  if (nprops > 2) nw_elim_range<NRV + 17, NRV + 12>(hh, g, y, dinv, l, adj[3] & 0x7u);
  if (nprops > 1) nw_elim_range<NRV + 11, NRV + 6>(hh, g, y, dinv, l, adj[2] & 0x3u);
  if (nprops > 0) nw_elim_range<NRV + 5, NRV>(hh, g, y, dinv, l, adj[1] & 0x1u);
  nw_elim_range<NRV - 1, 0>(hh, g, y, dinv, l, 0u);
  MRE_DBG_STAMP(4, 3);
#pragma unroll
  for (int k = 0; k < NV; k++)
    if (l <= k) s.W[k * (k + 1) / 2 + l] = hh[k];
  MRE_SYNC();
  {
    const int base = l < NV ? l * (l + 1) / 2 : 0;
    const int nva = NRV + 6 * nprops;
#pragma unroll
    for (int j = 0; j < NV - 1; j++) hh[j] = (j < l && l < nva) ? s.W[base + j] : 0.f;
#pragma unroll
    for (int j = 0; j < NV - 1; j++) {
      const float xj = rdlane(y * dinv, j);
      y = fmaf(-hh[j], xj, y);
    }
  }
  const float x = (l < NV && c.lact) ? y * dinv : 0.f;
  if (l < NVP) s.nw_search[l] = -x;
  const float dec = wave_sum((l < NVP ? s.nw_grad[l] : 0.f) * x);
  if (l == 0) s.scratch[2] = dec;
  MRE_SYNC();
  MRE_DBG_STAMP(4, 3);
}

MRE_PHASE_FN void nw_direction_reuse(ModelP M, Sm& s, int l) {
  const NwLane c = nw_lane(M, s, l);
  const int nva = NRV + 6 * s.nprops;
  const bool on = l < NV && c.lact;
  const float gin = on ? s.nw_grad[l] : 0.f;
  float g = gin;
  const float dinv = on ? 1.0f / s.W[l * (l + 1) / 2 + l] : 1.0f;
  float y = 0.f;
  for (int k = nva - 1; k >= 0; k--) {
    const float yk = rdlane(g * dinv, k);
    const float w = (l < k) ? s.W[k * (k + 1) / 2 + l] : 0.f;
    g = fmaf(-w, yk, g);
    y = (l == k) ? yk : y;
  }
  const int base = l < NV ? l * (l + 1) / 2 : 0;
  for (int j = 0; j < nva; j++) {
    const float cw = (j < l && l < NV) ? s.W[base + j] : 0.f;
    const float xj = rdlane(y * dinv, j);
    y = fmaf(-cw, xj, y);
  }
  const float x = on ? y * dinv : 0.f;
  if (l < NVP) s.nw_search[l] = -x;
  const float dec = wave_sum(gin * x);
  if (l == 0) s.scratch[2] = dec;
  MRE_SYNC();
}

template <bool PYR>
MRE_DEV float nw_search_move_impl(ModelP M, Sm& s, int l) {
  MRE_DBG_T0();
  const NwLane c = nw_lane(M, s, l);
  const int nefc = s.nefc, ncon = s.ncon, nscalar = 7 + s.nl;
  const float tol = M->opt_rec.tolerance, mu_scale = c.mu_scale;
  const bool on = l < NV && c.lact;
  const float fs = on ? s.qfrc_smooth[l] : 0.f, as = on ? s.qacc_smooth[l] : 0.f;
  float qa = on ? s.qacc[l] : 0.f, Ma = on ? s.nw_Ma[l] : 0.f;
  const float sv = on ? s.nw_search[l] : 0.f;
  const float Mv = on ? nw_mulM(s, l, c.mdiag, s.nw_search) : 0.f;
  for (int i = l; i < nefc; i += 64) s.jv[i] = row_dot(s, i, s.nw_search);
  MRE_SYNC();
  MRE_DBG_STAMP(7, 0);
  const float snorm = sqrtf(wave_sum(sv * sv));
  float alpha = 0.f;
#if defined(MRE_PHASE_STAMPS) && MRE_PHASE_STAMPS == 7
  int dbg_nev = 0;
#endif
  if (snorm >= kMinVal) {
    const float gtol_abs = tol * NW_LS_TOL * snorm / c.scale;
    float g0 = 0.5f * (Ma - fs) * (qa - as), g1 = sv * (Ma - fs), g2 = 0.5f * sv * Mv;
    wave_sum3(g0, g1, g2);
    float sq0 = 0.f, sq1 = 0.f, sq2 = 0.f, sj = 0.f, svv = 0.f;
    const bool s_on = l < nscalar, s_eq = l < 7;
    if (s_on) {
      const float D = 1.0f / s.efc_R[l];
      sj = s.jar[l]; svv = s.jv[l];
      sq0 = 0.5f * D * sj * sj; sq1 = D * sj * svv; sq2 = 0.5f * D * svv * svv;
    }
    float cq0 = 0.f, cq1 = 0.f, cq2 = 0.f, U0 = 0.f, V0 = 0.f, UU = 0.f, UV = 0.f, VV = 0.f, Dm = 0.f, mu = 0.f;
    const bool c_on = l < ncon;
    constexpr bool pyr = PYR;
    float pe0 = 0.f, pe1 = 0.f, pe2 = 0.f, pe3 = 0.f, pv0 = 0.f, pv1 = 0.f, pv2 = 0.f, pv3 = 0.f, pD = 0.f;
    if (c_on && pyr) {
      const int i = nscalar + 3 * l;
      const float fr = s.con_fric[l];
      const float j0 = s.jar[i], j1 = fr * s.jar[i + 1], j2 = fr * s.jar[i + 2];
      const float v0 = s.jv[i], v1 = fr * s.jv[i + 1], v2 = fr * s.jv[i + 2];
      pe0 = j0 + j1; pe1 = j0 - j1; pe2 = j0 + j2; pe3 = j0 - j2;
      pv0 = v0 + v1; pv1 = v0 - v1; pv2 = v0 + v2; pv3 = v0 - v2;
      pD = 1.0f / s.efc_R[i];
    }
    if (c_on && !pyr) {
      const int i = nscalar + 3 * l;
      const float fr = s.con_fric[l];
      mu = fr * mu_scale;
#pragma unroll
      for (int r = 0; r < 3; r++) {
        const float D = 1.0f / s.efc_R[i + r], j = s.jar[i + r], v = s.jv[i + r];
        cq0 += 0.5f * D * j * j; cq1 += D * j * v; cq2 += 0.5f * D * v * v;
      }
      const float U1 = s.jar[i + 1] * fr, U2 = s.jar[i + 2] * fr, V1 = s.jv[i + 1] * fr, V2 = s.jv[i + 2] * fr;
      U0 = s.jar[i] * mu; V0 = s.jv[i] * mu;
      UU = U1 * U1 + U2 * U2; UV = U1 * V1 + U2 * V2; VV = V1 * V1 + V2 * V2;
      Dm = (1.0f / s.efc_R[i]) / fmaxf(mu * mu * (1.f + mu * mu), kMinVal);
    }
#if defined(MRE_PHASE_STAMPS) && MRE_PHASE_STAMPS == 7
#define NW_DBG_EVAL() dbg_nev++
#else
#define NW_DBG_EVAL() do {} while (0)
#endif
    auto eval = [&](float a) {
      NW_DBG_EVAL();
      float q0 = 0.f, q1 = 0.f, q2 = 0.f, ec = 0.f, e1 = 0.f, e2 = 0.f;
      if (s_on && (s_eq || sj + a * svv < 0.f)) { q0 = sq0; q1 = sq1; q2 = sq2; }
      if (c_on && pyr) {
        const float x0 = fminf(pe0 + a * pv0, 0.f), x1 = fminf(pe1 + a * pv1, 0.f);
        const float x2 = fminf(pe2 + a * pv2, 0.f), x3 = fminf(pe3 + a * pv3, 0.f);
        ec = 0.5f * pD * ((x0 * x0 + x1 * x1) + (x2 * x2 + x3 * x3));
        e1 = pD * ((x0 * pv0 + x1 * pv1) + (x2 * pv2 + x3 * pv3));
        e2 = pD * (((x0 < 0.f ? pv0 * pv0 : 0.f) + (x1 < 0.f ? pv1 * pv1 : 0.f)) +
                   ((x2 < 0.f ? pv2 * pv2 : 0.f) + (x3 < 0.f ? pv3 * pv3 : 0.f)));
      }
      if (c_on && !pyr) {
        const float N = U0 + a * V0, Tsqr = UU + a * (2.f * UV + a * VV);
        bool quad = false;
        if (Tsqr <= 0.f) {
          quad = N < 0.f;
        } else {
          const float T = sqrtf(Tsqr);
          if (N >= mu * T) {
          } else if (mu * N + T <= 0.f) {
            quad = true;
          } else {
            const float iT = 1.0f / T;
            const float b = UV + a * VV;
            const float N1 = V0, T1 = b * iT, T2 = VV * iT - b * b * iT * iT * iT;
            const float NT = N - mu * T, w = N1 - mu * T1;
            ec = 0.5f * Dm * NT * NT;
            e1 = Dm * NT * w;
            e2 = Dm * (w * w - NT * mu * T2);
          }
        }
        if (quad) { q0 += cq0; q1 += cq1; q2 += cq2; }
      }
      NwPoint p;
      p.alpha = a;
      float s0 = ec + q0 + a * (q1 + a * q2), s1 = e1 + q1 + 2.f * a * q2, s2 = e2 + 2.f * q2;
      wave_sum3(s0, s1, s2);
      p.cost = s0 + g0 + a * (g1 + a * g2);
      p.d1 = s1 + g1 + 2.f * a * g2;
      p.d2 = s2 + 2.f * g2;
      return p;
    };
    const NwPoint p0 = eval(0.f);
    if (p0.d2 >= kMinVal) {
      const float gtol = fmaxf(gtol_abs, NW_LS_REL * fabsf(p0.d1));
      NwPoint p1 = eval(-p0.d1 / p0.d2);
      if (!(p1.cost <= p0.cost)) p1 = p0;
      if (fabsf(p1.d1) < gtol) {
        alpha = p1.alpha;
      } else {
        NwPoint lo = p0, hi = p0;
        bool have_lo = p0.d1 < 0.f, have_hi = !have_lo;
        bool found = false;
        for (int it = 0; it < NW_LS_MAX; it++) {
          if (p1.d1 < 0.f) { if (!have_lo || p1.alpha > lo.alpha) { lo = p1; have_lo = true; } }
          else { if (!have_hi || p1.alpha < hi.alpha) { hi = p1; have_hi = true; } }
          float a = p1.alpha - p1.d1 / p1.d2;
          if (have_lo && have_hi && !(a > lo.alpha && a < hi.alpha)) a = 0.5f * (lo.alpha + hi.alpha);
          if (fabsf(a - p1.alpha) <= 2e-7f * fabsf(p1.alpha)) break;
          p1 = eval(a);
          if (fabsf(p1.d1) < gtol) { found = true; break; }
        }
        if (found) alpha = p1.alpha;
        else if (have_lo && have_hi) alpha = lo.cost < hi.cost ? lo.alpha : hi.alpha;
        else alpha = p1.cost < p0.cost ? p1.alpha : 0.f;
      }
    }
  }
  if (l == 0) { s.scratch[0] = alpha; s.scratch[1] = 0.f; }
  MRE_DBG_STAMP(7, 1);
#if defined(MRE_PHASE_STAMPS) && MRE_PHASE_STAMPS == 7
  if (threadIdx.x == 0) dbg_acc[3] += (unsigned long long)dbg_nev << 4;
#endif
  if (alpha == 0.f) { MRE_SYNC(); return 0.f; }
  qa = fmaf(alpha, sv, qa);
  Ma = fmaf(alpha, Mv, Ma);
  if (l < NVP) { s.qacc[l] = qa; s.nw_Ma[l] = Ma; }
  for (int i = l; i < nefc; i += 64) s.jar[i] = fmaf(alpha, s.jv[i], s.jar[i]);
  MRE_SYNC();
  const float cost = nw_update_gradient<PYR>(s, l, c, nscalar, ncon);
  const float gr = l < NVP ? s.nw_grad[l] : 0.f;
  const float gn = sqrtf(wave_sum(gr * gr));
  if (l == 0) s.scratch[1] = gn;
  MRE_SYNC();
  MRE_DBG_STAMP(7, 2);
  return cost;
}
MRE_PHASE_FN float nw_search_move(ModelP M, Sm& s, int l) { return nw_search_move_impl<false>(M, s, l); }
MRE_PHASE_FN float nw_search_move_pyramidal(ModelP M, Sm& s, int l) { return nw_search_move_impl<true>(M, s, l); }

#ifdef MRE_PHASE_STAMPS
#define NW_STAMP(k)                                                          \
  do {                                                                       \
    const unsigned long long now_ = __builtin_amdgcn_s_memtime();            \
    if ((8 + (k)) / 4 == MRE_PHASE_STAMPS) stamp_acc[(k) % 4] += now_ - stamp_t; \
    stamp_t = now_;                                                          \
  } while (0)
MRE_DEV void newton_solve(ModelP M, Sm& s, int l, unsigned long long* stamp_acc, unsigned long long& stamp_t) {
#else
#define NW_STAMP(k) do {} while (0)
MRE_DEV void newton_solve(ModelP M, Sm& s, int l) {
#endif
  const float tol = M->opt_rec.tolerance;
  const int max_iter = M->opt_rec.iterations;
  const int nscalar = 7 + s.nl, ncon = s.ncon;
  float msum = M->opt_rec.M0_diag_robot_sum;
  for (int p = 0; p < s.nprops; p++)
    msum += 3.f * s.prop_mass[p] + s.prop_inertia[p][0] + s.prop_inertia[p][1] + s.prop_inertia[p][2];
  const float scale = 1.0f / msum;
  const bool pyr = M->opt_rec.cone == 0;
  if (pyr) nw_setup_pyramidal(M, s, l);
  else nw_setup(M, s, l);
  NW_STAMP(0);
#ifndef NW_TOL_FACTOR
#define NW_TOL_FACTOR 1.0f
#endif
  const float tol_eff = NW_TOL_FACTOR * tol;
  NwMasks mf = {0ull, 0ull, 0ull}, mprev = {~0ull, ~0ull, ~0ull};
  bool have_factor = false, force_full = false;
  float prev_dec = 3.0e38f;
  int iter = 0, nfull = 0, stalls = 0;
  while (iter < max_iter) {
    const NwMasks mk = nw_masks(s, l, nscalar, ncon);
    const bool reuse = have_factor && !force_full && mk == mf && mk.cc == 0ull;
    if (reuse) {
      nw_direction_reuse(M, s, l);
      NW_STAMP(2);
    } else {
      nw_direction(M, s, l);
      mf = mk; have_factor = true; nfull++;
      NW_STAMP(1);
    }
    const float dec = s.scratch[2];
    if (!(dec == dec)) break;
    if (0.5f * scale * dec < tol_eff) break;
    if (mk == mprev && dec > 0.1f * prev_dec) {
      if (reuse) { force_full = true; continue; }
      if (0.5f * scale * dec < 100.f * tol_eff && ++stalls >= 2) break;
    }
    prev_dec = dec; mprev = mk; force_full = false;
    if (pyr) nw_search_move_pyramidal(M, s, l);
    else nw_search_move(M, s, l);
    NW_STAMP(3);
    const float alpha = s.scratch[0];
    if (alpha == 0.f) {
      if (reuse) { force_full = true; continue; }
      break;
    }
    iter++;
    if (!reuse && mk.cc == 0ull && fabsf(alpha - 1.0f) < 1e-4f && nw_masks(s, l, nscalar, ncon) == mk) break;
  }
  if (l < NVP && !(l < NV)) s.qacc[l] = 0.f;
  if (l == 0) s.solver_iters = iter | (nfull << 8);
  MRE_SYNC();
}

MRE_DEV double rdlane_d(double v, int lane) {
  const long long b = __builtin_bit_cast(long long, v);
  const int lo = __builtin_amdgcn_readlane((int)(b & 0xFFFFFFFFll), lane);
  const int hi = __builtin_amdgcn_readlane((int)(b >> 32), lane);
  return __builtin_bit_cast(double, ((long long)hi << 32) | (long long)(unsigned)lo);
}
MRE_DEV double rcp_d(double x) {
  double r = __builtin_amdgcn_rcp(x);
  r = fma(fma(-x, r, 1.0), r, r);
  r = fma(fma(-x, r, 1.0), r, r);
  return r;
}
MRE_PHASE_FN bool nw_robot_polish(ModelP M, Sm& s, int l) {
  static_assert(offsetof(Sm, W) % 8 == 0 && offsetof(Sm, nw_Mv) % 8 == 0, "fp64 views of W / nw_Mv");
  constexpr int MAXROW = 7 + NRV;
  constexpr int NW_POLISH_CON = 32;
  static_assert(sizeof(((Sm*)0)->W) >= 8 * (2 * MAXROW + 10 * NW_POLISH_CON), "exchange area");
  static_assert(sizeof(((Sm*)0)->nw_Mv) >= 8 * NRV, "fp64 accelerations out");
  double* const frow = reinterpret_cast<double*>(&s.W[0]);
  double* const drow = frow + MAXROW;
  double* const fcon = drow + MAXROW;
  double* const a64 = reinterpret_cast<double*>(&s.nw_Mv[0]);
  const int nscalar = 7 + s.nl, ncon = s.ncon;
  constexpr int F0 = GRIP_BODY0 - 1;
  int nrc = 0;
  bool full = false;
  {
    const int rs = l < ncon ? (int)s.con_rslot[l] : HDR_NONE;
    const bool mine = rs != HDR_NONE;
    const unsigned long long m = __ballot(mine);
    nrc = __popcll(m);
    if (nrc > NW_POLISH_CON) return false;
    const int cb1 = mine ? (int)s.con_b1[l] : 0, cb2 = mine ? (int)s.con_b2[l] : 0;
    full = __ballot(mine && ((cb1 >= 1 && cb1 < GRIP_BODY0) || (cb2 >= 1 && cb2 < GRIP_BODY0))) != 0ull;
#ifdef MRE_POLISH_FULL
    full = true;
#endif
    if (mine) {
      const int k = __popcll(m & ((1ull << l) - 1ull));
      const int i = nscalar + 3 * l, h = s.hdr[i];
      const int pa = (h >> 8) & 0xF, pb = (h >> 12) & 0xF;
      double j[3], D[3];
#pragma unroll
      for (int r = 0; r < 3; r++) {
        double acc = -(double)s.efc_aref[i + r];
#pragma unroll
        for (int c = 0; c < NRV; c++) acc += (double)s.Jr[rs + r][c] * (double)s.qacc[c];
        if (pa < NPROP) { const float* ja = jpA(s, i + r); for (int c = 0; c < 6; c++) acc += (double)ja[c] * (double)s.qacc[NRV + 6 * pa + c]; }
        if (pb < NPROP) { const float* jb = jpB(s, i + r); for (int c = 0; c < 6; c++) acc += (double)jb[c] * (double)s.qacc[NRV + 6 * pb + c]; }
        j[r] = acc;
        D[r] = rcp_d((double)s.efc_R[i + r]);
      }
      const double fr = (double)s.con_fric[l], mu = fr * sqrt((double)s.efc_R[i + 1] / (double)s.efc_R[i]);
      const double U1 = j[1] * fr, U2 = j[2] * fr, Nn = j[0] * mu, T = sqrt(U1 * U1 + U2 * U2);
      double* o = fcon + 10 * k;
#pragma unroll
      for (int t = 0; t < 9; t++) o[t] = 0.0;
      o[9] = (double)rs;
      if (M->opt_rec.cone == 0) {
        const double e[4] = {j[0] + fr * j[1], j[0] - fr * j[1], j[0] + fr * j[2], j[0] - fr * j[2]};
        double a[4], n[4];
#pragma unroll
        for (int t = 0; t < 4; t++) { a[t] = e[t] < 0.0 ? e[t] : 0.0; n[t] = e[t] < 0.0 ? 1.0 : 0.0; }
        o[0] = -D[0] * (a[0] + a[1] + a[2] + a[3]);
        o[1] = -D[0] * fr * (a[0] - a[1]);
        o[2] = -D[0] * fr * (a[2] - a[3]);
        o[3] = D[0] * (n[0] + n[1] + n[2] + n[3]);
        o[4] = D[0] * fr * (n[0] - n[1]);
        o[5] = D[0] * fr * (n[2] - n[3]);
        o[6] = D[0] * fr * fr * (n[0] + n[1]);
        o[8] = D[0] * fr * fr * (n[2] + n[3]);
      } else if (Nn >= mu * T || (T <= 0.0 && Nn >= 0.0)) {
      } else if (mu * Nn + T <= 0.0 || (T <= 0.0 && Nn < 0.0)) {
        o[0] = -D[0] * j[0]; o[1] = -D[1] * j[1]; o[2] = -D[2] * j[2];
        o[3] = D[0]; o[6] = D[1]; o[8] = D[2];
      } else {
        const double Dm = D[0] / fmax(mu * mu * (1.0 + mu * mu), 1e-15), NT = Nn - mu * T, iT = 1.0 / T;
        o[0] = -Dm * NT * mu;
        o[1] = -o[0] * iT * U1 * fr;
        o[2] = -o[0] * iT * U2 * fr;
        const double a = mu * Nn * iT * iT * iT, dgn = mu * mu - mu * Nn * iT;
        o[3] = Dm * mu * mu;
        o[4] = Dm * mu * fr * (-mu * U1 * iT);
        o[5] = Dm * mu * fr * (-mu * U2 * iT);
        o[6] = Dm * fr * fr * (a * U1 * U1 + dgn);
        o[7] = Dm * fr * fr * (a * U1 * U2);
        o[8] = Dm * fr * fr * (a * U2 * U2 + dgn);
      }
    }
  }
  if (l < nscalar) {
    double jar = -(double)s.efc_aref[l];
#pragma unroll
    for (int j = 0; j < NRV; j++) jar += (double)s.Jr[l][j] * (double)s.qacc[j];
    const bool act = l < 7 || s.rstate[l] == NW_QUAD;
    const double D = act ? rcp_d((double)s.efc_R[l]) : 0.0;
    frow[l] = -D * jar;
    drow[l] = D;
  }
  MRE_SYNC();
  const int d = l < NRV ? l : 0;
  const bool row = l < NRV && (full || l >= F0);
  double hrow[NRV], g = 0.0;
#pragma unroll
  for (int j = 0; j < NRV; j++) hrow[j] = row ? (double)s.Md[d][j] : 0.0;
  if (row) {
    g = -(double)s.qfrc_smooth[d];
#pragma unroll
    for (int j = 0; j < NRV; j++) g += (double)s.Md[d][j] * (double)s.qacc[j];
    for (int r = 0; r < nscalar; r++) {
      const double jd = (double)s.Jr[r][d];
      g -= jd * frow[r];
      const double t = drow[r] * jd;
      if (full) {
#pragma unroll
        for (int j = 0; j < F0; j++) hrow[j] += t * (double)s.Jr[r][j];
      }
#pragma unroll
      for (int j = F0; j < NRV; j++) hrow[j] += t * (double)s.Jr[r][j];
    }
    for (int k = 0; k < nrc; k++) {
      const double* o = fcon + 10 * k;
      const int rs = (int)o[9];
      const double j0 = (double)s.Jr[rs][d], j1 = (double)s.Jr[rs + 1][d], j2 = (double)s.Jr[rs + 2][d];
      g -= j0 * o[0] + j1 * o[1] + j2 * o[2];
      const double t0 = j0 * o[3] + j1 * o[4] + j2 * o[5], t1 = j0 * o[4] + j1 * o[6] + j2 * o[7],
// ... 61 lines not shown
```

mujoco_robot_environments_amd/csrc/mre_solver.h:

```cpp
#pragma once

namespace mre {

constexpr int HDR_NONE = 0xFF;
constexpr int BLK_NONE = 0x7F;
constexpr int SCHED_NONE = 0xFF;
constexpr int TAB_OFF = MAXBLK * 5;
constexpr int TAB_ZEROS = 48;
static_assert(TAB_BYTES == 8 * (TAB_OFF + 1) + 4 * TAB_ZEROS, "operand table size");

#ifndef MRE_NEWTON
MRE_DEV void build_schedule(ModelP M, Sm& s);
#endif
MRE_DEV constexpr int cube_pair_bit(int p, int q) {
  const int a = p < q ? p : q, b = p < q ? q : p;
  return a == 0 ? b - 1 : (a == 1 ? b + 1 : 5);
}

MRE_DEV float prop_invM(const Sm& s, int p, int k) {
  return 1.0f / ((k < 3) ? s.prop_mass[p] : s.prop_inertia[p][k - 3]);
}

MRE_DEV void geom_pose(ModelP M, const Sm& s, int g, float* p, float* R, float* size,
                       float* rbound) {
  const int b = M->geom_body[g];
  float tmp[3], q[4];
  m3mulv(tmp, s.xmat[b], M->geom_pos[g]);
  v3add(p, s.xpos[b], tmp);
  qmul(q, s.xquat[b], M->geom_quat[g]);
  q2mat(R, q);
  const int pid = M->geom_propid[g];
  if (pid >= 0) {
    v3copy(size, s.prop_size[pid]);
    *rbound = v3norm(size);
  } else {
    v3copy(size, M->geom_size[g]);
    *rbound = M->geom_rbound[g];
  }
}

MRE_DEV void geom_center(ModelP M, const Sm& s, int g, float* p, float* rbound) {
  const int b = M->geom_body[g];
  float tmp[3];
  m3mulv(tmp, s.xmat[b], M->geom_pos[g]);
  v3add(p, s.xpos[b], tmp);
  const int pid = M->geom_propid[g];
  *rbound = pid >= 0 ? v3norm(s.prop_size[pid]) : M->geom_rbound[g];
}

MRE_PHASE_FN int collide_broad(ModelP M, Sm& s, int l, bool detect) {
  static_assert(offsetof(Sm, hdr) + sizeof(((Sm*)0)->hdr) - offsetof(Sm, JpA) >= sizeof(float) * 64 * COLL_BUF,
                "clip buffers do not fit");
  static_assert(NPAIR <= 256 && sizeof(((Sm*)0)->iscr) >= NPAIR, "survivor list: one byte per pair");
  MRE_DBG_T0();
  uint8_t* list = reinterpret_cast<uint8_t*>(s.iscr);
  const unsigned long long lt = (1ull << l) - 1ull;
  int nsurv = 0;
  for (int pass = 0; pass < NPAIR / 64; pass++) {
    const int pr = l + 64 * pass;
    const auto* R = &M->pair_rec[pr];
    const int g1 = R->g1, b1 = R->b1, b2 = R->b2, pid1 = R->pid1, pid2 = R->pid2, type1 = R->type1;
    const float lp1[3] = {R->pos1[0], R->pos1[1], R->pos1[2]}, lp2[3] = {R->pos2[0], R->pos2[1], R->pos2[2]};
    const float mrb1 = R->rb1, mrb2 = R->rb2, margin = R->margin, gap = R->gap;
    const float lq1[4] = {R->quat1[0], R->quat1[1], R->quat1[2], R->quat1[3]};
    bool live = false;
    if (g1 >= 0 && (pid1 < 0 || pid1 < s.nprops) && (pid2 < 0 || pid2 < s.nprops)) {
      const float inc = detect ? margin : margin - gap;
      float p1[3], p2[3], df[3], tmp[3];
      m3mulv(tmp, s.xmat[b1], lp1); v3add(p1, s.xpos[b1], tmp);
      m3mulv(tmp, s.xmat[b2], lp2); v3add(p2, s.xpos[b2], tmp);
      const float rb1 = pid1 >= 0 ? v3norm(s.prop_size[pid1]) : mrb1, rb2 = pid2 >= 0 ? v3norm(s.prop_size[pid2]) : mrb2;
      v3sub(df, p2, p1);
      if (type1 == 0) {
        float q[4], R1[9];
        qmul(q, s.xquat[b1], lq1);
        q2mat(R1, q);
        const float nn[3] = {R1[2], R1[5], R1[8]};
        live = v3dot(df, nn) - rb2 <= inc;
      } else {
        const float r = rb1 + rb2 + inc;
        live = v3dot(df, df) <= r * r;
      }
    }
    const unsigned long long m = __ballot(live);
    if (live) list[nsurv + __popcll(m & lt)] = (uint8_t)pr;
    nsurv += __popcll(m);
  }
  if (l == 0) s.ncon = 0;
  MRE_SYNC();
  MRE_DBG_STAMP(6, 0);
  return nsurv;
}
MRE_PHASE_FN int collide_narrow(ModelP M, Sm& s, int l, bool detect, bool clip_always, int c0, int nsurv, int base) {
  MRE_DBG_T0();
  float* buf = &s.JpA[0][0] + l * COLL_BUF;
  const uint8_t* list = reinterpret_cast<const uint8_t*>(s.iscr);
  const unsigned long long lt = (1ull << l) - 1ull;
  {
    const int pr = (c0 + l < nsurv) ? list[c0 + l] : -1;
    float normal[3] = {0.f, 0.f, 1.f};
    int n = 0;
    FaceCand rc;
    unsigned rm = 0u;
    if (pr >= 0) {
      const auto* R = &M->pair_rec[pr];
      const int b1 = R->b1, b2 = R->b2, pid1 = R->pid1, pid2 = R->pid2, type1 = R->type1;
      const float lp1[3] = {R->pos1[0], R->pos1[1], R->pos1[2]}, lp2[3] = {R->pos2[0], R->pos2[1], R->pos2[2]};
      const float lq1[4] = {R->quat1[0], R->quat1[1], R->quat1[2], R->quat1[3]};
      const float lq2[4] = {R->quat2[0], R->quat2[1], R->quat2[2], R->quat2[3]};
      const float ms1[3] = {R->size1[0], R->size1[1], R->size1[2]}, ms2[3] = {R->size2[0], R->size2[1], R->size2[2]};
      const float margin = R->margin, gap = R->gap;
      float p1[3], R1[9], s1[3], p2[3], R2[9], s2[3], tmp[3], q[4];
      m3mulv(tmp, s.xmat[b1], lp1); v3add(p1, s.xpos[b1], tmp);
      qmul(q, s.xquat[b1], lq1); q2mat(R1, q);
      m3mulv(tmp, s.xmat[b2], lp2); v3add(p2, s.xpos[b2], tmp);
      qmul(q, s.xquat[b2], lq2); q2mat(R2, q);
      if (pid1 >= 0) v3copy(s1, s.prop_size[pid1]); else v3copy(s1, ms1);
      if (pid2 >= 0) v3copy(s2, s.prop_size[pid2]); else v3copy(s2, ms2);
      const float inc = detect ? margin : margin - gap;
      MRE_DBG_STAMP(6, 1);
      if ((R->single >> 8) == 2) n = cyl_box(p1, R1, s1, p2, R2, s2[0], s2[2], inc, normal, buf);
      else if (type1 == 0) n = plane_box(p1, R1, p2, R2, s2, inc, normal, buf);
      else n = box_box(p1, R1, s1, p2, R2, s2, inc, normal, buf, clip_always, rc, rm);
      MRE_DBG_STAMP(6, 2);
      int m = 0;
      if (rm & FACE_IN_REGS) {
#pragma unroll
        for (int v = 0; v < 4; v++) {
          if (((rm >> v) & 1u) != 0u && rc.d[v] < inc) m++;
          else rm &= ~(1u << v);
        }
      } else {
        for (int c = 0; c < n; c++)
          if (cand_dist(buf, c) < inc) {
            if (m != c) {
              for (int k = 0; k < 3; k++) cand_xyz(buf, m)[k] = cand_xyz(buf, c)[k];
              cand_dist(buf, m) = cand_dist(buf, c);
            }
            m++;
          }
      }
      n = m;
    }
#if defined(MRE_PHASE_STAMPS) && MRE_PHASE_STAMPS == 8
    {
      const bool tbl = pr >= 0 && (M->pair_rec[pr].g1 == 1);
      const unsigned long long fb = __ballot((rm & FACE_BRANCH) != 0u), fr = __ballot((rm & FACE_IN_REGS) != 0u), tb = __ballot(tbl);
      if (l == 0) {
        dbg_acc[0] += (unsigned long long)__popcll(fb) << 4; dbg_acc[1] += (unsigned long long)__popcll(fr) << 4;
        dbg_acc[2] += (unsigned long long)__popcll(fb & tb) << 4; dbg_acc[3] += (unsigned long long)__popcll(fr & tb) << 4;
      }
    }
#endif
    const bool single = pr >= 0 && n > 1 && (M->pair_rec[pr].single & 0xFF) != 0;
    const int ncand = n;
    if (single) n = 1;
    int off = base, tot = base;
    for (int bit = 0; bit < 4; bit++) {
      const unsigned long long m = __ballot((n >> bit) & 1);
      off += __popcll(m & lt) << bit;
      tot += __popcll(m) << bit;
    }
    if (l == 0) {
      s.ncon = tot < NCON_MAX ? tot : NCON_MAX;
      if (tot > NCON_MAX) s.overflow = 1;
    }
    if (single) {
      const float incw = M->pair_rec[pr].margin - M->pair_rec[pr].gap;
      if (rm & FACE_IN_REGS) {
        float wsum = 0.f, px = 0.f, py = 0.f, pz = 0.f, dmin = 0.f, bx = 0.f, by = 0.f, bz = 0.f;
        bool first = true;
#pragma unroll
        for (int v = 0; v < 4; v++)
          if (((rm >> v) & 1u) != 0u) {
            const float dc = rc.d[v];
            if (first || dc < dmin) { dmin = dc; bx = rc.x[v]; by = rc.y[v]; bz = rc.z[v]; }
            first = false;
            const float w = incw - dc;
            if (w > 0.f) { wsum += w; px += w * rc.x[v]; py += w * rc.y[v]; pz += w * rc.z[v]; }
          }
        if (wsum > 0.f) { const float iw = 1.0f / wsum; px *= iw; py *= iw; pz *= iw; }
        else { px = bx; py = by; pz = bz; }
        rc.x[0] = px; rc.y[0] = py; rc.z[0] = pz; rc.d[0] = dmin;
        rm = FACE_IN_REGS | 1u;
      } else {
        float wsum = 0.f, px = 0.f, py = 0.f, pz = 0.f, dmin = cand_dist(buf, 0);
        int best = 0;
        for (int c = 0; c < ncand; c++) {
          const float dc = cand_dist(buf, c);
          if (dc < dmin) { dmin = dc; best = c; }
          const float w = incw - dc;
          if (w > 0.f) { wsum += w; px += w * cand_xyz(buf, c)[0]; py += w * cand_xyz(buf, c)[1]; pz += w * cand_xyz(buf, c)[2]; }
        }
        if (wsum > 0.f) { const float iw = 1.0f / wsum; px *= iw; py *= iw; pz *= iw; }
        else { px = cand_xyz(buf, best)[0]; py = cand_xyz(buf, best)[1]; pz = cand_xyz(buf, best)[2]; }
        cand_xyz(buf, 0)[0] = px; cand_xyz(buf, 0)[1] = py; cand_xyz(buf, 0)[2] = pz;
        cand_dist(buf, 0) = dmin;
      }
    }
    if (n > 0) {
      float f[9];
      v3copy(f, normal);
      make_frame(f);
      if (rm & FACE_IN_REGS) {
        int id = off;
#pragma unroll
        for (int v = 0; v < 4; v++)
          if (((rm >> v) & 1u) != 0u && id < NCON_MAX) {
            s.con_pos[id][0] = rc.x[v]; s.con_pos[id][1] = rc.y[v]; s.con_pos[id][2] = rc.z[v];
            for (int k = 0; k < 9; k++) s.con_frame[id][k] = f[k];
            s.con_dist[id] = rc.d[v];
            s.con_pair[id] = (uint8_t)pr;
            id++;
          }
      } else {
        for (int c = 0; c < n; c++) {
          const int id = off + c;
          if (id >= NCON_MAX) break;
          const float cx0 = cand_xyz(buf, c)[0], cx1 = cand_xyz(buf, c)[1], cx2 = cand_xyz(buf, c)[2];
          s.con_pos[id][0] = cx0; s.con_pos[id][1] = cx1; s.con_pos[id][2] = cx2;
          for (int k = 0; k < 9; k++) s.con_frame[id][k] = f[k];
          s.con_dist[id] = cand_dist(buf, c);
          s.con_pair[id] = (uint8_t)pr;
        }
      }
    }
    MRE_SYNC();
    MRE_DBG_STAMP(6, 3);
    return tot;
  }
}
MRE_DEV void collide(ModelP M, Sm& s, int l, bool detect, bool clip_always) {
  const int nsurv = collide_broad(M, s, l, detect);
  int base = 0;
  for (int c0 = 0; c0 < nsurv; c0 += 64) {
    base = collide_narrow(M, s, l, detect, clip_always, c0, nsurv, base);
    if (base > NCON_MAX) break;
  }
}

MRE_DEV float impedance(const float* solimp, float pos, float margin) {
  const float dmin = clampf(solimp[0], 0.0001f, 0.9999f), dmax = clampf(solimp[1], 0.0001f, 0.9999f);
  const float width = fmaxf(solimp[2], kMinVal), mid = clampf(solimp[3], 0.0001f, 0.9999f);
  const float power = fmaxf(solimp[4], 1.0f);
  if (dmin == dmax) return 0.5f * (dmin + dmax);
  const float x = fabsf((pos - margin) / width);
  if (x >= 1.0f) return dmax;
  if (x <= 0.0f) return dmin;
  float y;
  if (power == 1.0f) y = x;
  else if (power == 2.0f) {
    y = (x <= mid) ? x * x / mid : 1.0f - (1.0f - x) * (1.0f - x) / (1.0f - mid);
  }
  else if (x <= mid) y = powf(x, power) / powf(mid, power - 1.0f);
  else y = 1.0f - powf(1.0f - x, power) / powf(1.0f - mid, power - 1.0f);
  return dmin + y * (dmax - dmin);
}

MRE_DEV void jac_robot(ModelP M, Sm& s, int rs, int b, const float* p, const float* ax, float sg) {
  float off[3];
  v3sub(off, p, s.com_robot);
  const int n = M->chain_len[b];
  for (int k = 0; k < n; k++) {
    const int j = M->chain_dof[b][k];
    const float* c = s.cdof[j];
    float t[3];
    v3cross(t, c, off);
    s.Jr[rs][j] += sg * (ax[0] * (c[3] + t[0]) + ax[1] * (c[4] + t[1]) + ax[2] * (c[5] + t[2]));
  }
}
MRE_DEV int row_blk(const Sm& s, int i, int& r) {
  const int ns = 7 + s.nl;
  if (i < ns) { r = i % 3; return i / 3; }
  const int cr = i - ns;
  r = cr % 3;
  return 8 + cr / 3;
}
#ifdef MRE_NEWTON
MRE_DEV float& rowR(Sm& s, int i) { return s.efc_R[i]; }
MRE_DEV float& rowB(Sm& s, int i) { return s.efc_aref[i]; }
#else
MRE_DEV float& rowR(Sm& s, int i) { int r; const int b = row_blk(s, i, r); return s.blkrec[b][r]; }
MRE_DEV float& rowB(Sm& s, int i) { int r; const int b = row_blk(s, i, r); return s.blkrec[b][3 + r]; }
MRE_DEV float& rowAinv(Sm& s, int i) { int r; const int b = row_blk(s, i, r); return s.blkrec[b][6 + r]; }
#endif

MRE_DEV float* jpA(Sm& s, int i) { return s.JpA[i - 7 - s.nl]; }
MRE_DEV const float* jpA(const Sm& s, int i) { return s.JpA[i - 7 - s.nl]; }
MRE_DEV float* jpB(Sm& s, int i) { const int cr = i - 7 - s.nl; return s.JpB[3 * s.con_bslot[cr / 3] + cr % 3]; }
MRE_DEV const float* jpB(const Sm& s, int i) { const int cr = i - 7 - s.nl; return s.JpB[3 * s.con_bslot[cr / 3] + cr % 3]; }
MRE_DEV void jac_prop(Sm& s, int i, int slot, int b, const float* p, const float* ax, float sg) {
  float off[3];
  v3sub(off, p, s.xpos[b]);
  float* J = slot == 0 ? jpA(s, i) : jpB(s, i);
  for (int k = 0; k < 3; k++) {
    J[k] = sg * ax[k];
    float axk[3] = {s.xmat[b][k], s.xmat[b][3 + k], s.xmat[b][6 + k]}, t[3];
    v3cross(t, axk, off);
    J[3 + k] = sg * v3dot(ax, t);
  }
}

MRE_DEV float row_dot(const Sm& s, int i, const float* vec) {
  const int h = s.hdr[i];
  const int rs = h & 0xFF, pa = (h >> 8) & 0xF, pb = (h >> 12) & 0xF;
  float acc = 0.f;
  if (rs != HDR_NONE)
    for (int j = 0; j < NRV; j++) acc += s.Jr[rs][j] * vec[j];
  if (pa < NPROP)
    { const float* ja = jpA(s, i); for (int k = 0; k < 6; k++) acc += ja[k] * vec[NRV + 6 * pa + k]; }
  if (pb < NPROP)
    { const float* jb = jpB(s, i); for (int k = 0; k < 6; k++) acc += jb[k] * vec[NRV + 6 * pb + k]; }
  return acc;
}

MRE_DEV void row_dot2(const Sm& s, int i, const float* v1, const float* v2, float& r1, float& r2) {
  const int h = s.hdr[i];
  const int rs = h & 0xFF, pa = (h >> 8) & 0xF, pb = (h >> 12) & 0xF;
  float a1 = 0.f, a2 = 0.f;
  if (rs != HDR_NONE)
    for (int j = 0; j < NRV; j++) { const float jv = s.Jr[rs][j]; a1 += jv * v1[j]; a2 += jv * v2[j]; }
  if (pa < NPROP) {
    const float* ja = jpA(s, i);
    for (int k = 0; k < 6; k++) { const float jv = ja[k]; a1 += jv * v1[NRV + 6 * pa + k]; a2 += jv * v2[NRV + 6 * pa + k]; }
  }
  if (pb < NPROP) {
    const float* jb = jpB(s, i);
    for (int k = 0; k < 6; k++) { const float jv = jb[k]; a1 += jv * v1[NRV + 6 * pb + k]; a2 += jv * v2[NRV + 6 * pb + k]; }
  }
  r1 = a1; r2 = a2;
}

#ifndef MRE_NEWTON
MRE_PHASE_FN void solve_robot_rows(Sm& s, int l) {
  for (int rs = l; rs < s.nrrow; rs += 64) {
    float x[NRV];
#pragma unroll
    for (int k = 0; k < NRV; k++) x[k] = s.Jr[rs][k];
    solve_robot_regs(s.qLD, s.qLDinv, x);
#pragma unroll
    for (int k = 0; k < NRV; k++) s.Br[rs][k] = x[k];
  }
  MRE_SYNC();
}

#endif

constexpr int GRIP0 = GRIP_BODY0;

MRE_PHASE_FN void assemble_constraints(ModelP M, Sm& s, int l) {
  int lim = 0, lim_side = 0;
  const auto* BR = &M->body_rec[l < NRB ? l : 0];
  const int jnt_limited = BR->jnt_limited;
  const float jnt_range[2] = {BR->jnt_range[0], BR->jnt_range[1]};
  if (l >= 1 && l < NRB && jnt_limited) {
    const double q = robot_q(s, l - 1);
    if (q - (double)jnt_range[0] < 0.0) { lim = 1; lim_side = -1; }
    else if ((double)jnt_range[1] - q < 0.0) { lim = 1; lim_side = 1; }
  }
  keep_live(jnt_range[0]); keep_live(jnt_range[1]);
  const unsigned long long limm = __ballot(lim != 0);
  const int lim_idx = __popcll(limm & ((1ull << l) - 1ull));
  if (l == 0) s.nl = __popcll(limm);
  if (lim) s.lim_info[lim_idx] = l | ((lim_side > 0 ? 1 : 0) << 8);
  if (l < s.ncon) {
    const int pr = s.con_pair[l];
    s.con_b1[l] = (uint8_t)M->pair_rec[pr].b1;
    s.con_b2[l] = (uint8_t)M->pair_rec[pr].b2;
  }
  MRE_SYNC();
#ifndef MRE_NEWTON
  {
    static_assert(sizeof(s.sched) % 4 == 0, "schedule cleared by words");
    unsigned* w = reinterpret_cast<unsigned*>(&s.sched[0][0]);
    for (int e = l; e < (int)(sizeof(s.sched) / 4); e += 64) w[e] = 0x01010101u * (unsigned)SCHED_NONE;
  }
#endif
  {
    const int base = 7 + s.nl, ncon0 = s.ncon;
    const bool on = l < ncon0;
    const int cb1 = on ? s.con_b1[l] : 0, cb2 = on ? s.con_b2[l] : 0;
    const bool rob_any = on && ((cb1 < NRB && cb1 > 0) || (cb2 < NRB && cb2 > 0));
    const bool fing = on && ((cb1 >= GRIP_BODY0 && cb1 < NRB) || (cb2 >= GRIP_BODY0 && cb2 < NRB));
    const unsigned long long fingm = __ballot(fing);
    const bool two_props = on && cb1 >= NRB && cb2 >= NRB;
    const unsigned long long lt = (1ull << l) - 1ull;
    const unsigned long long rmask = __ballot(rob_any), tmask = __ballot(two_props);
    const int my_r = base + 3 * __popcll(rmask & lt), my_b = __popcll(tmask & lt);
    const bool fail = on && (base + 3 * (l + 1) > NEFC_MAX || (rob_any && my_r + 3 > NRROW_MAX) ||
                             (two_props && my_b >= NPP_MAX));
    const unsigned long long fmask = __ballot(fail);
    const int kept = fmask != 0ull ? (int)__builtin_ctzll(fmask) : ncon0;
    if (l < kept) {
      s.con_rslot[l] = rob_any ? my_r : HDR_NONE;
      s.con_bslot[l] = two_props ? my_b : 0;
    }
    MRE_SYNC();
    if (l == 0) {
      const unsigned long long below = kept >= 64 ? ~0ull : ((1ull << kept) - 1ull);
      if (fmask != 0ull) s.overflow = 1;
      s.ncon = kept;
      s.nefc = base + 3 * kept;
      s.nrrow = base + 3 * __popcll(rmask & below);
      s.npp = __popcll(tmask & below);
      s.finger_contact = (fingm & below) != 0ull;
#ifdef MRE_NEWTON
      s.nsched = 0; s.nblk = 0;
#else
      build_schedule(M, s);
#endif
    }
  }
  MRE_SYNC();
  const int nefc = s.nefc, nl = s.nl;
  for (int e = l; e < s.nrrow * NRV; e += 64) (&s.Jr[0][0])[e] = 0.f;
#ifndef MRE_NEWTON
  for (int e = l; e < 8 * 16; e += 64) (&s.blkrec[0][0])[e] = 0.f;
#endif
  MRE_SYNC();
  for (int i = l; i < nefc; i += 64) {
    int rs = HDR_NONE, pa = 0xF, pb = 0xF;
    float pos = 0.f, margin = 0.f, diag = 0.f, imp_pos = 0.f;
    bool fric_row = false;
    float R0scale = 1.0f;
    const int eqi = i < 6 ? i / 3 : 2;
    const int limb = (i >= 7 && i < 7 + nl) ? (s.lim_info[i - 7] & 0xFF) : 0;
    const int rrec = i < 7 ? eqi : (i < 7 + nl ? ROWREC_JNT + limb : ROWREC_PAIR + s.con_pair[(i - 7 - nl) / 3]);
    const auto* RR = &M->row_rec[rrec];
    const float solref[2] = {RR->solref[0], RR->solref[1]};
    const float solimp[5] = {RR->solimp[0], RR->solimp[1], RR->solimp[2], RR->solimp[3], RR->solimp[4]};
    const float rec_margin = RR->margin, rec_gap = RR->gap, rec_friction = RR->friction, invw1 = RR->invw1, invw2 = RR->invw2;
    const float lim_range[2] = {M->body_rec[limb].jnt_range[0], M->body_rec[limb].jnt_range[1]};
    const float opt_timestep = M->opt_rec.timestep, opt_impratio = M->opt_rec.impratio;
    const int opt_cone = M->opt_rec.cone;
    if (i < 7) {
      rs = i;
      const int e = eqi;
      const auto* E = &M->eq_rec[e];
      const int b1 = E->b1, b2 = E->b2;
      const int root = E->root, pb1 = E->pb1, pb2 = E->pb2;
      const float pc[5] = {E->data[0], E->data[1], E->data[2], E->data[3], E->data[4]};
      const float q0_1 = E->qpos0_1, q0_2 = E->qpos0_2;
      const int nchain = E->root_chain_len;
      int chain[MAXCHAIN];
#pragma unroll
      for (int c = 0; c < MAXCHAIN; c++) chain[c] = E->root_chain[c];
      if (e < 2) {
        const int k = i % 3;
        const float* loc = &s.qfrc_con[16 * e];
        const float* R = s.xmat[root];
        float cp[3];
        m3mulv(cp, R, loc);
        const float rk[3] = {R[3 * k], R[3 * k + 1], R[3 * k + 2]};
        s.Jr[rs][b1 - 1] += v3dot(rk, loc + 4);
        if (pb1 >= GRIP0) s.Jr[rs][pb1 - 1] += v3dot(rk, loc + 7);
        s.Jr[rs][b2 - 1] += v3dot(rk, loc + 10);
        if (pb2 >= GRIP0) s.Jr[rs][pb2 - 1] += v3dot(rk, loc + 13);
        {
#pragma unroll
          for (int c = 0; c < MAXCHAIN; c++) {
            if (c < nchain) {
              const int j = chain[c];
              float t[3];
              v3cross(t, s.cdof[j], cp);
              s.Jr[rs][j] += sel3(t, k);
            }
          }
        }
        pos = sel3(cp, k);
        imp_pos = v3norm(cp);
        diag = invw1 + invw2;
      } else {
        const int d1 = b1 - 1, d2 = b2 - 1;
        const double dif64 = robot_q(s, d2) - (double)q0_2;
        pos = (float)(robot_q(s, d1) - (double)q0_1 -
                      ((double)pc[0] + dif64 * ((double)pc[1] + dif64 * ((double)pc[2] + dif64 * ((double)pc[3] + dif64 * (double)pc[4])))));
        const float dif = (float)dif64;
        const float deriv = pc[1] + dif * (2.f * pc[2] + dif * (3.f * pc[3] + dif * 4.f * pc[4]));
        s.Jr[rs][d1] += 1.f;
        s.Jr[rs][d2] -= deriv;
        imp_pos = pos;
        diag = invw1 + invw2;
      }
      keep_live(root); keep_live(pb1); keep_live(pb2); keep_live(nchain); keep_live(q0_1); keep_live(q0_2);
#pragma unroll
      for (int c = 0; c < 5; c++) keep_live(pc[c]);
#pragma unroll
      for (int c = 0; c < MAXCHAIN; c++) keep_live(chain[c]);
    } else if (i < 7 + nl) {
      rs = i;
      const int info = s.lim_info[i - 7], b = info & 0xFF, hi = (info >> 8) & 1;
      const double q = robot_q(s, b - 1);
      pos = (float)(hi ? ((double)lim_range[1] - q) : (q - (double)lim_range[0]));
      s.Jr[rs][b - 1] = hi ? -1.f : 1.f;
      imp_pos = pos;
      diag = invw1;
    } else {
      const int c = (i - 7 - nl) / 3, r = (i - 7 - nl) % 3;
      const int b1 = s.con_b1[c], b2 = s.con_b2[c];
      const float* ax = &s.con_frame[c][3 * r];
      const float* p = s.con_pos[c];
      const int rs0 = s.con_rslot[c];
      if (rs0 != HDR_NONE) rs = rs0 + r;
      int slot = 0;
      float dg = 0.f;
      if (b1 > 0) {
        if (b1 < NRB) { jac_robot(M, s, rs, b1, p, ax, -1.f); dg += invw1; }
        else { pa = b1 - NRB; jac_prop(s, i, slot++, b1, p, ax, -1.f); dg += 1.0f / s.prop_mass[pa]; }
      }
      if (b2 > 0) {
        if (b2 < NRB) { jac_robot(M, s, rs, b2, p, ax, 1.f); dg += invw2; }
        else {
          const int pid = b2 - NRB;
          if (slot == 0) pa = pid; else pb = pid;
          jac_prop(s, i, slot++, b2, p, ax, 1.f);
          dg += 1.0f / s.prop_mass[pid];
        }
      }
      diag = dg;
      margin = rec_margin - rec_gap;
      imp_pos = s.con_dist[c];
      if (r == 0) pos = s.con_dist[c];
      else {
        fric_row = true;
        pos = 0.f;
        R0scale = 1.0f / fmaxf(opt_impratio, kMinVal);
      }
      if (opt_cone == 0) {
        const float fr = rec_friction;
        diag = dg * (1.f + fr * fr);
        R0scale = 2.f * fr * fr / fmaxf(opt_impratio, kMinVal);
      }
    }
    keep_live(lim_range[0]); keep_live(lim_range[1]); keep_live(invw1); keep_live(invw2); keep_live(rec_friction);
    keep_live(rec_margin); keep_live(rec_gap); keep_live(opt_impratio); keep_live(opt_cone);
    s.hdr[i] = rs | (pa << 8) | (pb << 12);
    const float imp = impedance(solimp, imp_pos, margin);
    float tc = solref[0];
    const float dr = solref[1], dmax = clampf(solimp[1], 0.0001f, 0.9999f);
    float K, B;
    if (tc > 0.f) {
      tc = fmaxf(tc, 2.f * opt_timestep);
      K = 1.0f / (dmax * dmax * tc * tc * dr * dr);
      B = 2.0f / (dmax * tc);
    } else { K = -tc / (dmax * dmax); B = -dr / dmax; }
    if (fric_row) K = 0.f;
    float R = fmaxf((1.f - imp) * diag / imp, kMinVal) * R0scale;
    if (opt_cone == 0) R = fmaxf(R, kMinVal);
    const float vel = row_dot(s, i, s.qvel);
    const float efc_margin = fric_row ? 0.f : margin;
    const float aref = -B * vel - K * imp * (pos - efc_margin);
    rowR(s, i) = R; rowB(s, i) = aref;
#ifdef MRE_NEWTON
    if (i >= 7 + nl && (i - 7 - nl) % 3 == 0) s.con_fric[(i - 7 - nl) / 3] = rec_friction;
#else
    if (i >= 7 + nl && (i - 7 - nl) % 3 == 0) s.blkrec[8 + (i - 7 - nl) / 3][15] = rec_friction;
#endif
  }
  MRE_SYNC();
}

#ifndef MRE_NEWTON
MRE_PHASE_FN void assemble_blocks(ModelP M, Sm& s, int l) {
  const int nefc = s.nefc, nl = s.nl;
  for (int i = l; i < nefc; i += 64) {
    const int h = s.hdr[i];
    const int rs = h & 0xFF, pa = (h >> 8) & 0xF, pb = (h >> 12) & 0xF;
    const bool scalar = i < 7 + nl;
    const int r = scalar ? i % 3 : (i - 7 - nl) % 3;
    const int i0 = i - r;
    const int nb = scalar ? ((7 + nl - i0) < 3 ? (7 + nl - i0) : 3) : 3;
    const int slot = scalar ? i / 3 : 8 + (i - 7 - nl) / 3;
    float acc[3] = {0.f, 0.f, 0.f};
#pragma unroll
    for (int cc = 0; cc < 3; cc++) {
      float a = 0.f;
      if (cc < nb) {
        if (rs != HDR_NONE) {
          const int rs2 = rs - r + cc;
          for (int j = 0; j < NRV; j++) a += s.Jr[rs][j] * s.Br[rs2][j];
        }
        if (pa < NPROP)
          { const float *x = jpA(s, i), *y = jpA(s, i0 + cc); for (int k = 0; k < 6; k++) a += x[k] * y[k] * prop_invM(s, pa, k); }
        if (pb < NPROP)
          { const float *x = jpB(s, i), *y = jpB(s, i0 + cc); for (int k = 0; k < 6; k++) a += x[k] * y[k] * prop_invM(s, pb, k); }
      }
      acc[cc] = a;
    }
    const float diag = (r == 0 ? acc[0] : (r == 1 ? acc[1] : acc[2])) + rowR(s, i);
    if (r == 0) acc[0] = scalar ? acc[0] : diag;
    if (r == 1) acc[1] = scalar ? acc[1] : diag;
    if (r == 2) acc[2] = scalar ? acc[2] : diag;
    if (r == 0) { s.blkrec[slot][9] = acc[0]; s.blkrec[slot][10] = acc[1]; s.blkrec[slot][11] = acc[2]; }
    if (r == 1) { s.blkrec[slot][12] = acc[1]; s.blkrec[slot][13] = acc[2]; }
    if (r == 2) { s.blkrec[slot][14] = acc[2]; }
    s.blkrec[slot][6 + r] = 1.0f / diag;
  }
  MRE_SYNC();
}

MRE_DEV float fast_rcp(float x) { return __builtin_amdgcn_rcpf(x); }

MRE_DEV bool qcqp2(float* res, const float* A, const float* b, float d0, float d1, float r) {
  const float b1 = b[0] * d0, b2 = b[1] * d1;
  const float A11 = A[0] * d0 * d0, A22 = A[3] * d1 * d1, A12 = A[1] * d0 * d1;
  float la = 0.f, v1 = 0.f, v2 = 0.f;
  const float r2 = r * r;
  for (int iter = 0; iter < 20; iter++) {
    const float det = (A11 + la) * (A22 + la) - A12 * A12;
    if (det < 1e-10f) { res[0] = res[1] = 0.f; return false; }
    const float di = fast_rcp(det);
    const float P11 = (A22 + la) * di, P22 = (A11 + la) * di, P12 = -A12 * di;
    v1 = -P11 * b1 - P12 * b2;
    v2 = -P12 * b1 - P22 * b2;
    const float val = v1 * v1 + v2 * v2 - r * r;
    if (val < fmaxf(1e-10f, 1e-6f * r2)) break;
    const float deriv = -2.0f * (P11 * v1 * v1 + 2.0f * P12 * v1 * v2 + P22 * v2 * v2);
    const float delta = -val * fast_rcp(deriv);
    if (delta < 1e-10f) break;
    la += delta;
  }
  res[0] = v1 * d0;
  res[1] = v2 * d1;
  return la != 0.f;
}

MRE_DEV int lane_island(int l) { return l < 16 ? 0 : (l < 48 ? 1 + ((l - 16) >> 3) : -1); }
MRE_DEV int lane_dof(int l) {
  if (l < NRV) return l;
  if (l >= 16 && l < 48 && ((l - 16) & 7) < 6) return NRV + 6 * ((l - 16) >> 3) + ((l - 16) & 7);
  return -1;
}
MRE_DEV void island_sum3(float& x, float& y, float& z) {
  asm volatile(
      "s_nop 1\n\t"
      "v_add_f32_dpp %0, %0, %0 quad_perm:[1,0,3,2] row_mask:0xf bank_mask:0xf bound_ctrl:1\n\t"
      "v_add_f32_dpp %1, %1, %1 quad_perm:[1,0,3,2] row_mask:0xf bank_mask:0xf bound_ctrl:1\n\t"
      "v_add_f32_dpp %2, %2, %2 quad_perm:[1,0,3,2] row_mask:0xf bank_mask:0xf bound_ctrl:1\n\t"
      "v_add_f32_dpp %0, %0, %0 quad_perm:[2,3,0,1] row_mask:0xf bank_mask:0xf bound_ctrl:1\n\t"
      "v_add_f32_dpp %1, %1, %1 quad_perm:[2,3,0,1] row_mask:0xf bank_mask:0xf bound_ctrl:1\n\t"
      "v_add_f32_dpp %2, %2, %2 quad_perm:[2,3,0,1] row_mask:0xf bank_mask:0xf bound_ctrl:1\n\t"
      "v_add_f32_dpp %0, %0, %0 row_half_mirror row_mask:0xf bank_mask:0xf bound_ctrl:1\n\t"
      "v_add_f32_dpp %1, %1, %1 row_half_mirror row_mask:0xf bank_mask:0xf bound_ctrl:1\n\t"
      "v_add_f32_dpp %2, %2, %2 row_half_mirror row_mask:0xf bank_mask:0xf bound_ctrl:1\n\t"
      "v_add_f32_dpp %0, %0, %0 row_mirror row_mask:0x1 bank_mask:0xf\n\t"
      "v_add_f32_dpp %1, %1, %1 row_mirror row_mask:0x1 bank_mask:0xf\n\t"
      "v_add_f32_dpp %2, %2, %2 row_mirror row_mask:0x1 bank_mask:0xf\n\t"
      "s_nop 1"
      : "+v"(x), "+v"(y), "+v"(z));
}

MRE_DEV void lane_JB(const Sm& s, int row, int rs, int l, int lk, int slot, float linvM, float& j, float& b) {
  j = 0.f; b = 0.f;
  if (l < NRV) {
    if (rs != BLK_NONE) { j = s.Jr[rs][l]; b = s.Br[rs][l]; }
  } else if (slot >= 0) {
    j = (slot == 0 ? jpA(s, row) : jpB(s, row))[lk];
    b = j * linvM;
  }
}


MRE_DEV void build_schedule(ModelP M, Sm& s) {
  int* last = s.iscr;
  for (int k = 0; k < 5; k++) last[k] = 0;
  const int nscalar = 7 + s.nl;
  int nb = 0, nst = 0;
  for (int i = 0; i < nscalar; i += 3) {
    Blk b;
    b.row0 = (uint16_t)i; b.type = 0; b.nrows = (uint8_t)((nscalar - i) < 3 ? (nscalar - i) : 3);
    b.rslot = (uint8_t)i; b.pa = 0xF; b.pb = 0xF; b.primary = 0; b.bslot = 0;
    const int st = last[0]++;
    s.sched[st][0] = (uint8_t)nb;
    s.blk[nb++] = b;
    if (last[0] > nst) nst = last[0];
  }
  for (int c = 0; c < s.ncon; c++) {
    const int b1 = s.con_b1[c], b2 = s.con_b2[c];
    const int rs = s.con_rslot[c];
    int pa = 0xF, pb = 0xF;
    if (b1 >= NRB) pa = b1 - NRB;
    if (b2 >= NRB) { if (pa == 0xF) pa = b2 - NRB; else pb = b2 - NRB; }
    const bool hr = rs != HDR_NONE, ha = pa != 0xF, hb = pb != 0xF;
    int st = 0;
    if (hr && last[0] > st) st = last[0];
    if (ha && last[1 + pa] > st) st = last[1 + pa];
    if (hb && last[1 + pb] > st) st = last[1 + pb];
    Blk b;
// ... 419 lines not shown
```

mujoco_robot_environments_amd/lib.py:

```python
from __future__ import annotations

import ctypes as C
import os
import shutil
import subprocess
from typing import Optional

_CSRC = os.path.join(os.path.dirname(os.path.abspath(__file__)), "csrc")
_SO = os.path.join(_CSRC, "libmre.so")
_SOURCES = ["mre_kernels.hip", "mre_render.hip", "mre_api.cpp"]
_HEADERS = ["mre_dev.h", "mre_math.h", "mre_collide.h", "mre_solver.h", "mre_newton.h", "mre_osc.h",
            os.path.join("..", "..", "include", "mre.h")]
_UNHASHED_SOURCES = ["mre_records.hip", "mre_records.h", "mre_labels.hip", "mre_labels.h", "mre_heightmap.hip", "mre_heightmap.h",
                     "mre_heightmap_point.h", "mre_warp.hip", "mre_warp.h", "mre_warp_point.h", "mre_model.cpp", "mre_model.h", "mre_sched.cpp", "mre_env.h",
                     "mre_policy.h", "mre_launch.h"]
_LIB: Optional[C.CDLL] = None

MRE_NQ, MRE_NV, MRE_NU, MRE_NQ_PAD, MRE_NV_PAD, MRE_MAX_PROPS = 43, 39, 8, 44, 40, 4
MRE_TRACE_W = 88
MRE_TRACE_QVEL = 48
MRE_FINAL_W = 83
MRE_DYN_W = 128

EXPORTS = [
    "mre_create", "mre_destroy", "mre_last_error", "mre_num_envs", "mre_stream", "mre_sync",
    "mre_set_props", "mre_reset", "mre_place_props", "mre_set_state", "mre_get_state", "mre_get_ctrl",
    "mre_set_warmstart", "mre_get_warmstart", "mre_set_ctrl", "mre_step", "mre_rollout", "mre_rollout_ticks",
    "mre_set_trace", "mre_osc_set_target", "mre_osc_configure", "mre_gripper_set",
    "mre_run_controller", "mre_get_sites", "mre_get_status", "mre_get_solver_stats",
    "mre_profile_enable", "mre_profile_read", "mre_set_env_id_offset", "mre_set_env_order",
    "mre_set_fallback", "mre_get_fallback_stats", "mre_get_queue_info", "mre_set_solver", "mre_get_solver", "mre_wait_stream", "mre_osc_compute", "mre_get_contacts", "mre_get_contacts_full", "mre_get_settle_steps", "mre_get_launch_info", "mre_prop_place", "mre_sort_colours", "mre_crc32c", "mre_osc_configure_env", "mre_set_env_ids", "mre_set_render_colours", "mre_render",
    "mre_get_state_f64", "mre_set_state_f64", "mre_get_time", "mre_pack_final_state",
    "mre_records_workspace_bytes", "mre_varint_pack_rows", "mre_crc32c_rows", "mre_crc32c_combine",
    "mre_varint_unpack_workspace_bytes", "mre_varint_unpack_rows", "mre_get_arm_dynamics", "mre_seg_labels",
    "mre_heightmap", "mre_warp_maps",
]
MRE_UNPACK_LONG, MRE_UNPACK_OVERFLOW, MRE_UNPACK_TRUNCATED, MRE_UNPACK_COUNT, MRE_UNPACK_DESC = 1, 2, 4, 8, 16


class MreError(RuntimeError):
    pass


def source_hash() -> str:
    import hashlib
    h = hashlib.sha256()
    for f in sorted(f for f in _SOURCES + _HEADERS if not f.endswith(("mre_api.cpp", "mre.h"))):
        with open(os.path.join(_CSRC, f), "rb") as fh:
            h.update(f.encode() + b"\0" + fh.read())
    return h.hexdigest()[:16]


def needs_build() -> bool:
    if not os.path.exists(_SO):
        return True
    t = os.path.getmtime(_SO)
    for f in _SOURCES + _HEADERS + _UNHASHED_SOURCES:
        p = os.path.join(_CSRC, f)
        if os.path.exists(p) and os.path.getmtime(p) > t:
            return True
    return False


def build(force: bool = False, verbose: bool = False) -> str:
    if not force and not needs_build():
        return _SO
    hipcc = shutil.which("hipcc") or "/opt/rocm/bin/hipcc"
    base = [hipcc, "--offload-arch=gfx950", "-O3", "-std=c++17", "-fPIC", "-Wno-unused-value", "-ffp-contract=on",
            "-fno-hip-fp32-correctly-rounded-divide-sqrt"]
    if verbose:
        base.insert(1, "-Rpass-analysis=kernel-resource-usage")
    bdir = os.path.join(_CSRC, "_build")
    os.makedirs(bdir, exist_ok=True)
    units = [("kernels", "mre_kernels.hip", []), ("kernels_large", "mre_kernels.hip", ["-DMRE_LARGE_CAPS"]),
             ("kernels_newton", "mre_kernels.hip", ["-DMRE_NEWTON"]),
             ("kernels_large_newton", "mre_kernels.hip", ["-DMRE_LARGE_CAPS", "-DMRE_NEWTON"]),
             ("render", "mre_render.hip", []), ("records", "mre_records.hip", []),
             ("labels", "mre_labels.hip", []), ("heightmap", "mre_heightmap.hip", []),
             ("warp", "mre_warp.hip", []), ("api", "mre_api.cpp", []),
             ("sched", "mre_sched.cpp", []), ("model", "mre_model.cpp", [])]
    procs = [(name, subprocess.Popen(base + flags + ["-c", os.path.join(_CSRC, src), "-o",
                                                     os.path.join(bdir, name + ".o")]))
             for name, src, flags in units]
    for name, pr in procs:
        if pr.wait() != 0:
            raise MreError(f"hipcc failed on translation unit {name}")
    subprocess.check_call([hipcc, "--offload-arch=gfx950", "-shared", "-fPIC", "-o", _SO] +
                          [os.path.join(bdir, name + ".o") for name, _, _ in units])
    return _SO


def lib() -> C.CDLL:
    global _LIB
    if _LIB is not None:
        return _LIB
    import torch
    so = os.environ.get("MRE_LIB", _SO)
    if not os.path.exists(so):
        raise MreError(f"{so} is missing: run `python -c 'import __graft_entry__ as g; g.build()'` "
                       "(the HIP extension is the only implementation of the step)")
    L = C.CDLL(so)
    vp, ci, cu, fp = C.c_void_p, C.c_int, C.c_uint, C.c_void_p
    L.mre_create.argtypes = [C.c_char_p, C.c_size_t, ci, ci, C.POINTER(vp)]
    L.mre_destroy.argtypes = [vp]
    L.mre_last_error.restype = C.c_char_p
    L.mre_num_envs.argtypes = [vp]
    L.mre_stream.restype = vp
    L.mre_stream.argtypes = [vp]
    L.mre_sync.argtypes = [vp]
    L.mre_set_props.argtypes = [vp, fp, fp]
    L.mre_reset.argtypes = [vp, fp]
    L.mre_place_props.argtypes = [vp, fp, C.c_uint64, fp, fp, ci, ci]
    L.mre_set_state.argtypes = [vp, fp, fp]
    L.mre_get_state.argtypes = [vp, fp, fp]
    L.mre_get_state_f64.argtypes = [vp, fp, fp]
    L.mre_set_state_f64.argtypes = [vp, fp, fp]
    L.mre_get_time.argtypes = [vp, fp]
    L.mre_get_ctrl.argtypes = [vp, fp]
    L.mre_set_warmstart.argtypes = [vp, fp]
    L.mre_get_warmstart.argtypes = [vp, fp]
    L.mre_set_ctrl.argtypes = [vp, fp]
    L.mre_step.argtypes = [vp, ci, cu]
    L.mre_rollout.argtypes = [vp, fp, ci, ci, cu]
    L.mre_rollout_ticks.argtypes = [vp, fp, ci, ci, cu, ci]
    L.mre_pack_final_state.argtypes = [vp, fp]
    L.mre_set_trace.argtypes = [vp, fp, ci, ci]
    L.mre_osc_set_target.argtypes = [vp, fp, fp, fp, fp, fp]
    L.mre_osc_configure.argtypes = [vp, fp, fp, fp, ci]
    L.mre_gripper_set.argtypes = [vp, fp]
    L.mre_run_controller.argtypes = [vp, ci, ci, fp]
    L.mre_get_sites.argtypes = [vp, fp, fp, fp]
    L.mre_get_status.argtypes = [vp, fp]
    L.mre_get_solver_stats.argtypes = [vp, fp]
    L.mre_set_env_id_offset.argtypes = [vp, C.c_longlong]
    L.mre_set_env_ids.argtypes = [vp, C.POINTER(C.c_longlong)]
    L.mre_set_env_order.argtypes = [vp, fp]
    L.mre_profile_enable.argtypes = [vp, ci]
    L.mre_profile_read.argtypes = [vp, C.POINTER(C.c_float), C.POINTER(ci)]
    L.mre_set_fallback.argtypes = [vp, ci]
    L.mre_set_solver.argtypes = [vp, ci]
    L.mre_get_solver.argtypes = [vp]
    L.mre_wait_stream.argtypes = [vp, vp]
    L.mre_osc_compute.argtypes = [vp, fp, fp]
    L.mre_get_arm_dynamics.argtypes = [vp, ci, fp]
    L.mre_get_contacts.argtypes = [vp, fp, fp]
    L.mre_get_contacts_full.argtypes = [vp, ci, fp, fp]
    L.mre_get_settle_steps.argtypes = [vp, fp]
    L.mre_get_launch_info.argtypes = [vp, fp]
    L.mre_prop_place.argtypes = [vp, C.c_uint64, fp, fp, fp, ci, C.c_float, fp, fp]
    L.mre_sort_colours.argtypes = [vp, C.c_uint64, fp, fp, ci, C.c_float, fp, fp, fp, fp]
    L.mre_set_render_colours.argtypes = [vp, fp, fp]
    L.mre_render.argtypes = [vp, fp, fp, C.c_float, ci, ci, fp, fp, fp, fp]
    L.mre_osc_configure_env.argtypes = [vp, fp, fp, fp]
    L.mre_get_fallback_stats.argtypes = [vp, C.POINTER(C.c_longlong)]
    L.mre_get_queue_info.argtypes = [vp, C.POINTER(C.c_longlong)]
    sz = C.c_size_t
    L.mre_crc32c.restype = C.c_uint32
    L.mre_crc32c.argtypes = [C.c_char_p, sz]
    L.mre_crc32c_combine.restype = C.c_uint32
    L.mre_crc32c_combine.argtypes = [C.c_uint32, C.c_uint32, sz]
    L.mre_records_workspace_bytes.restype = sz
    L.mre_records_workspace_bytes.argtypes = [ci, sz]
    L.mre_varint_pack_rows.argtypes = [vp, fp, sz, sz, fp, ci, ci, fp, sz, fp, fp, fp, fp, sz]
    L.mre_crc32c_rows.argtypes = [vp, fp, sz, sz, fp, ci, ci, fp, fp, sz]
# ... 19 lines not shown
```

Measured before the change: 25.19 million.

## Pack dof chains into nibble records and software-pipeline Newton Hessian gathers

Replaces the per-body chain_len/chain_dof tables with a 16-byte packed ChainRec (a nibble per dof) that is loaded once per constraint row. The Jacobian accumulation now writes instead of read-modify-writing on the first contribution. Broadphase pair records are hoisted into registers before the pass loop, and narrowphase record fields are loaded once. The Newton direction's MFMA accumulation loop now prefetches the next chunk's gather one step ahead by default, with the old serial schedule kept behind MRE_NEWTON_SERIAL. The aim is to cut scattered model-memory loads and hide gather latency, at the cost of higher register pressure.

```diff
diff --git a/mujoco_robot_environments_amd/csrc/mre_api.cpp b/mujoco_robot_environments_amd/csrc/mre_api.cpp
--- a/mujoco_robot_environments_amd/csrc/mre_api.cpp
+++ b/mujoco_robot_environments_amd/csrc/mre_api.cpp
@@ -70,6 +70,7 @@
   { int rc = sched_create(e); if (rc) return rc; }
   if (const char* fb = getenv("MRE_NO_FALLBACK")) e->fallback = atoi(fb) == 0;
   if (const char* ng = getenv("MRE_NARROW_GENERIC")) e->base_flags = atoi(ng) != 0 ? F_CLIP_ALWAYS : 0u;
+  if (const char* ns = getenv("MRE_NEWTON_SERIAL")) e->base_flags |= atoi(ns) != 0 ? F_NW_SERIAL : 0u;
   if (const char* fl = getenv("MRE_FORCE_LARGE")) {
     if (atoi(fl) != 0) {
       e->h_large.assign(N, 1); e->n_large = num_envs;
diff --git a/mujoco_robot_environments_amd/csrc/mre_dev.h b/mujoco_robot_environments_amd/csrc/mre_dev.h
--- a/mujoco_robot_environments_amd/csrc/mre_dev.h
+++ b/mujoco_robot_environments_amd/csrc/mre_dev.h
@@ -127,6 +127,8 @@
   int root_chain[12];
 };
 static_assert(sizeof(EqRec) == 128 && MAXCHAIN <= 12, "EqRec is eight 16-byte words");
+struct alignas(16) ChainRec { uint32_t w[4]; };
+static_assert(sizeof(ChainRec) == 16 && MAXCHAIN <= 16 && NRV <= 16, "ChainRec: a nibble per dof of the chain");
 struct alignas(16) SiteRec {
   float pos[3]; int body;
   float quat[4];
@@ -145,8 +147,6 @@
 
 struct DevModel {
   int body_propid[NB];
-  int chain_len[NB];
-  int chain_dof[NB][MAXCHAIN];
   float body_mass[NB];
   int dof_Madr[NV + 1];
   float qpos0[NQP];
@@ -164,6 +164,7 @@
   MEntryRec m_rec[NMR];
   RowRec row_rec[NROWREC];
   EqRec eq_rec[NEQ];
+  ChainRec chain_rec[NRB];
   SiteRec site_rec[NSITE];
   OptRec opt_rec;
 };
@@ -177,7 +178,7 @@
 
 enum StepFlags : unsigned { F_NO_CONSTRAINTS = 1u, F_FREEZE_ROBOT = 2u, F_CONV_CONTINUE = 4u, F_CONV_OPEN = 8u,
                             F_OSC_EVAL = 16u, F_DETECT = 32u, F_SETTLE_EXIT = 64u, F_DETECT_ACTIVE = 128u,
-                            F_CLIP_ALWAYS = 256u };
+                            F_CLIP_ALWAYS = 256u, F_NW_SERIAL = 512u };
 enum CtrlMode : int { CTRL_HELD = 0, CTRL_SEQ = 1, CTRL_OSC = 2 };
 
 struct StepArgs {
diff --git a/mujoco_robot_environments_amd/csrc/mre_jac_point.h b/mujoco_robot_environments_amd/csrc/mre_jac_point.h
--- /dev/null
+++ b/mujoco_robot_environments_amd/csrc/mre_jac_point.h
@@ -0,0 +1,38 @@
+#ifndef MRE_JAC_POINT_H
+#define MRE_JAC_POINT_H
+#include <stdint.h>
+
+#if defined(__HIP__)
+#define MRE_JP_HD __host__ __device__
+#else
+#define MRE_JP_HD
+#endif
+
+constexpr int JP_MAXCHAIN = 16;
+
+MRE_JP_HD inline bool jp_chain_pack(uint32_t* w, const int* dof, int n) {
+  w[0] = w[1] = w[2] = w[3] = 0u;
+  if (n < 0 || n > JP_MAXCHAIN) return false;
+  for (int k = 0; k < n; k++) {
+    if (dof[k] < 0 || dof[k] > 15) return false;
+    w[1 + (k >> 3)] |= (uint32_t)dof[k] << (4 * (k & 7));
+  }
+  w[0] = (uint32_t)n;
+  return true;
+}
+MRE_JP_HD inline int jp_chain_len(const uint32_t* w) { return (int)w[0]; }
+MRE_JP_HD inline uint64_t jp_chain_bits(const uint32_t* w) { return (uint64_t)w[1] | ((uint64_t)w[2] << 32); }
+MRE_JP_HD inline int jp_chain_dof(const uint32_t* w, int k) { return (int)((jp_chain_bits(w) >> (4 * k)) & 15u); }
+
+MRE_JP_HD inline bool jp_chain_same(const uint32_t* w, const int* dof, int n) {
+  uint32_t x[4];
+  if (!jp_chain_pack(x, dof, n)) return false;
+  return w[0] == x[0] && w[1] == x[1] && w[2] == x[2] && w[3] == x[3];
+}
+
+MRE_JP_HD inline float jp_term(const float* c, const float* off, const float* ax, float sg) {
+  float x = c[1] * off[2] - c[2] * off[1], y = c[2] * off[0] - c[0] * off[2], z = c[0] * off[1] - c[1] * off[0];
+  return sg * (ax[0] * (c[3] + x) + ax[1] * (c[4] + y) + ax[2] * (c[5] + z));
+}
+MRE_JP_HD inline float jp_accumulate(float entry, float term, bool first) { return (first ? 0.f : entry) + term; }
+#endif
diff --git a/mujoco_robot_environments_amd/csrc/mre_kernels.hip b/mujoco_robot_environments_amd/csrc/mre_kernels.hip
--- a/mujoco_robot_environments_amd/csrc/mre_kernels.hip
+++ b/mujoco_robot_environments_amd/csrc/mre_kernels.hip
@@ -2,6 +2,7 @@
 
 #include "mre_dev.h"
 #include "mre_math.h"
+#include "mre_jac_point.h"
 #include "mre_collide.h"
 
 namespace mre {
@@ -1451,10 +1452,10 @@
     bool polished = false;
     if (constrained) {
 #if defined(MRE_NEWTON) && defined(MRE_PHASE_STAMPS)
-      newton_solve(M, s, l, stamp_acc, stamp_t);
+      newton_solve(M, s, l, a.flags, stamp_acc, stamp_t);
       polished = nw_robot_polish(M, s, l);
 #elif defined(MRE_NEWTON)
-      newton_solve(M, s, l);
+      newton_solve(M, s, l, a.flags);
       polished = nw_robot_polish(M, s, l);
 #else
       if (M->opt_rec.cone == 0) solve_constraints_pyramidal(M, s, l);
diff --git a/mujoco_robot_environments_amd/csrc/mre_model.cpp b/mujoco_robot_environments_amd/csrc/mre_model.cpp
--- a/mujoco_robot_environments_amd/csrc/mre_model.cpp
+++ b/mujoco_robot_environments_amd/csrc/mre_model.cpp
@@ -1,4 +1,5 @@
 #include "mre_model.h"
+#include "mre_jac_point.h"
 
 #include <cstdint>
 #include <cstring>
@@ -112,6 +113,8 @@
     q.root_chain_len = t.chain_len[q.root];
     for (int c = 0; c < MAXCHAIN; c++) q.root_chain[c] = t.chain_dof[q.root][c];
   }
+  for (int b = 0; b < NRB; b++)
+    if (!jp_chain_pack(m.chain_rec[b].w, t.chain_dof[b], t.chain_len[b])) return "a robot body's dof chain does not fit its record";
   for (int b = 1; b < NRB; b++) {
     RowRec& r = m.row_rec[ROWREC_JNT + b];
     for (int c = 0; c < 2; c++) r.solref[c] = t.jnt_solref[b][c];
@@ -200,6 +203,16 @@
     ok = ok && q.root == root;
     SAME(q.root_chain_len, t.chain_len[root]);
     for (int c = 0; c < MAXCHAIN; c++) SAME(q.root_chain[c], t.chain_dof[root][c]);
+  }
+  for (int b = 0; b < NRB && ok; b++) {
+    const ChainRec& r = m.chain_rec[b];
+    ok = ok && jp_chain_len(r.w) == t.chain_len[b] && t.chain_len[b] <= MAXCHAIN;
+    for (int k = 0; k < t.chain_len[b] && ok; k++) ok = ok && jp_chain_dof(r.w, k) == t.chain_dof[b][k];
+    ok = ok && jp_chain_same(r.w, t.chain_dof[b], t.chain_len[b]);
+    if (b >= 1 && ok) {
+      ok = t.chain_len[b] >= 1 && t.chain_dof[b][t.chain_len[b] - 1] == t.body_dofadr[b] && t.dof_parent[t.chain_dof[b][0]] == -1;
+      for (int k = 1; k < t.chain_len[b] && ok; k++) ok = t.dof_parent[t.chain_dof[b][k]] == t.chain_dof[b][k - 1];
+    }
   }
   for (int b = 1; b < NRB && ok; b++) {
     const RowRec& r = m.row_rec[ROWREC_JNT + b];
@@ -367,7 +380,7 @@
     t.park_pos[p][0] = 2.0f + 0.5f * p; t.park_pos[p][1] = 2.0f; t.park_pos[p][2] = -5.0f;
   }
 #define KEEP(x) static_assert(sizeof(m.x) == sizeof(t.x), #x); memcpy(&m.x, &t.x, sizeof(m.x))
-  KEEP(body_propid); KEEP(chain_len); KEEP(chain_dof); KEEP(body_mass);
+  KEEP(body_propid); KEEP(body_mass);
   KEEP(dof_Madr); KEEP(qpos0); KEEP(M_i); KEEP(M_j);
   KEEP(geom_type); KEEP(geom_body); KEEP(geom_propid); KEEP(geom_size); KEEP(geom_pos); KEEP(geom_quat); KEEP(geom_rbound);
   KEEP(pair_g1); KEEP(pair_g2); KEEP(pair_margin);
diff --git a/mujoco_robot_environments_amd/csrc/mre_newton.h b/mujoco_robot_environments_amd/csrc/mre_newton.h
--- a/mujoco_robot_environments_amd/csrc/mre_newton.h
+++ b/mujoco_robot_environments_amd/csrc/mre_newton.h
@@ -338,7 +338,8 @@
 MRE_PHASE_FN float nw_setup(ModelP M, Sm& s, int l) { return nw_setup_impl<false>(M, s, l); }
 MRE_PHASE_FN float nw_setup_pyramidal(ModelP M, Sm& s, int l) { return nw_setup_impl<true>(M, s, l); }
 
-MRE_PHASE_FN void nw_direction(ModelP M, Sm& s, int l) {
+MRE_PHASE_FN void nw_direction(ModelP M, Sm& s, int l, unsigned flags) {
+  const bool serial = (flags & F_NW_SERIAL) != 0;
   MRE_DBG_T0();
   const NwLane c = nw_lane(M, s, l);
   const int nefc = s.nefc, nscalar = 7 + s.nl, nprops = s.nprops;
@@ -387,13 +388,12 @@
     };
     static_assert(sizeof(s.Jr[0]) == 60 && sizeof(s.JpA[0]) == 24 && sizeof(s.JpB[0]) == 24, "row strides of the gathers");
     struct Meta { int ii, st, h; float R; uint2 d; };
-    auto chunk = [&](const Meta& cur, Meta& nxt, int r0) {
+    auto operands = [&](const Meta& cur, bool pre, float p0, float p1, float p2,
+                        float& v0, float& v1, float& v2, float& a0, float& a1, float& a2) {
       const int ii = cur.ii, h = cur.h, st = cur.st;
       const uint2 d = cur.d;
       const bool quad = st == NW_QUAD, cone = st == NW_CONE;
       const float D = quad ? __builtin_amdgcn_rcpf(cur.R) : 0.f;
-      if (r0 + 4 < nefc) meta(r0 + 4, nxt.ii, nxt.st, nxt.h, nxt.R, nxt.d);
-      float v0, v1, v2, a0, a1, a2;
       if (__any(cone)) {
         const int cr = ii - nscalar;
         const int k = cone ? cr % 3 : 0;
@@ -413,9 +413,12 @@
         a1 = cone ? H0 * x1 + H1 * y1 + H2 * z1 : v1 * D;
         a2 = cone ? H0 * x2 + H1 * y2 + H2 * z2 : v2 * D;
       } else {
-        gather(h, d, v0, v1, v2);
+        if (pre) { v0 = p0; v1 = p1; v2 = p2; }
+        else gather(h, d, v0, v1, v2);
         a0 = v0 * D; a1 = v1 * D; a2 = v2 * D;
       }
+    };
+    auto issue = [&](float a0, float a1, float a2, float v0, float v1, float v2) {
       c00 = __builtin_amdgcn_mfma_f32_16x16x4f32(a0, v0, c00, 0, 0, 0);
       c10 = __builtin_amdgcn_mfma_f32_16x16x4f32(a1, v0, c10, 0, 0, 0);
       c11 = __builtin_amdgcn_mfma_f32_16x16x4f32(a1, v1, c11, 0, 0, 0);
@@ -425,12 +428,37 @@
         c22 = __builtin_amdgcn_mfma_f32_16x16x4f32(a2, v2, c22, 0, 0, 0);
       }
     };
-    Meta mA, mB;
-    meta(0, mA.ii, mA.st, mA.h, mA.R, mA.d);
-    mB = mA;
-    for (int r0 = 0; r0 < nefc; r0 += 8) {
-      chunk(mA, mB, r0);
-      if (r0 + 4 < nefc) chunk(mB, mA, r0 + 4);
+    if (serial) {
+      auto chunk = [&](const Meta& cur, Meta& nxt, int r0) {
+        if (r0 + 4 < nefc) meta(r0 + 4, nxt.ii, nxt.st, nxt.h, nxt.R, nxt.d);
+        float v0, v1, v2, a0, a1, a2;
+        operands(cur, false, 0.f, 0.f, 0.f, v0, v1, v2, a0, a1, a2);
+        issue(a0, a1, a2, v0, v1, v2);
+      };
+      Meta mA, mB;
+      meta(0, mA.ii, mA.st, mA.h, mA.R, mA.d);
+      mB = mA;
+      for (int r0 = 0; r0 < nefc; r0 += 8) {
+        chunk(mA, mB, r0);
+        if (r0 + 4 < nefc) chunk(mB, mA, r0 + 4);
+      }
+    } else {
+      Meta m0, m1, m2;
+      meta(0, m0.ii, m0.st, m0.h, m0.R, m0.d);
+      m1 = m0;
+      if (4 < nefc) meta(4, m1.ii, m1.st, m1.h, m1.R, m1.d);
+      m2 = m1;
+      float g0, g1, g2;
+      gather(m0.h, m0.d, g0, g1, g2);
+      for (int r0 = 0; r0 < nefc; r0 += 4) {
+        if (r0 + 8 < nefc) meta(r0 + 8, m2.ii, m2.st, m2.h, m2.R, m2.d);
+        float n0 = 0.f, n1 = 0.f, n2 = 0.f;
+        if (r0 + 4 < nefc) gather(m1.h, m1.d, n0, n1, n2);
+        float v0, v1, v2, a0, a1, a2;
+        operands(m0, true, g0, g1, g2, v0, v1, v2, a0, a1, a2);
+        issue(a0, a1, a2, v0, v1, v2);
+        m0 = m1; m1 = m2; g0 = n0; g1 = n1; g2 = n2;
+      }
     }
     MRE_DBG_STAMP(4, 1);
     float* T = s.W;
@@ -711,10 +739,10 @@
     if ((8 + (k)) / 4 == MRE_PHASE_STAMPS) stamp_acc[(k) % 4] += now_ - stamp_t; \
     stamp_t = now_;                                                          \
   } while (0)
-MRE_DEV void newton_solve(ModelP M, Sm& s, int l, unsigned long long* stamp_acc, unsigned long long& stamp_t) {
+MRE_DEV void newton_solve(ModelP M, Sm& s, int l, unsigned flags, unsigned long long* stamp_acc, unsigned long long& stamp_t) {
 #else
 #define NW_STAMP(k) do {} while (0)
-MRE_DEV void newton_solve(ModelP M, Sm& s, int l) {
+MRE_DEV void newton_solve(ModelP M, Sm& s, int l, unsigned flags) {
 #endif
   const float tol = M->opt_rec.tolerance;
   const int max_iter = M->opt_rec.iterations;
@@ -742,7 +770,7 @@
       nw_direction_reuse(M, s, l);
       NW_STAMP(2);
     } else {
-      nw_direction(M, s, l);
+      nw_direction(M, s, l, flags);
       mf = mk; have_factor = true; nfull++;
       NW_STAMP(1);
     }
diff --git a/mujoco_robot_environments_amd/csrc/mre_solver.h b/mujoco_robot_environments_amd/csrc/mre_solver.h
--- a/mujoco_robot_environments_amd/csrc/mre_solver.h
+++ b/mujoco_robot_environments_amd/csrc/mre_solver.h
@@ -56,13 +56,24 @@
   uint8_t* list = reinterpret_cast<uint8_t*>(s.iscr);
   const unsigned long long lt = (1ull << l) - 1ull;
   int nsurv = 0;
+  struct BroadRec { int g1, b1, b2, pid1, pid2, type1; float lp1[3], lp2[3], mrb1, mrb2, margin, gap, lq1[4]; };
+  BroadRec rec[NPAIR / 64];
+#pragma unroll
+  for (int pass = 0; pass < NPAIR / 64; pass++) {
+    const auto* R = &M->pair_rec[l + 64 * pass];
+    BroadRec& r = rec[pass];
+    r.g1 = R->g1; r.b1 = R->b1; r.b2 = R->b2; r.pid1 = R->pid1; r.pid2 = R->pid2; r.type1 = R->type1;
+    for (int k = 0; k < 3; k++) { r.lp1[k] = R->pos1[k]; r.lp2[k] = R->pos2[k]; }
+    r.mrb1 = R->rb1; r.mrb2 = R->rb2; r.margin = R->margin; r.gap = R->gap;
+    for (int k = 0; k < 4; k++) r.lq1[k] = R->quat1[k];
+  }
+#pragma unroll
   for (int pass = 0; pass < NPAIR / 64; pass++) {
     const int pr = l + 64 * pass;
-    const auto* R = &M->pair_rec[pr];
-    const int g1 = R->g1, b1 = R->b1, b2 = R->b2, pid1 = R->pid1, pid2 = R->pid2, type1 = R->type1;
-    const float lp1[3] = {R->pos1[0], R->pos1[1], R->pos1[2]}, lp2[3] = {R->pos2[0], R->pos2[1], R->pos2[2]};
-    const float mrb1 = R->rb1, mrb2 = R->rb2, margin = R->margin, gap = R->gap;
-    const float lq1[4] = {R->quat1[0], R->quat1[1], R->quat1[2], R->quat1[3]};
+    const BroadRec& r = rec[pass];
+    const int g1 = r.g1, b1 = r.b1, b2 = r.b2, pid1 = r.pid1, pid2 = r.pid2, type1 = r.type1;
+    const float* lp1 = r.lp1; const float* lp2 = r.lp2; const float* lq1 = r.lq1;
+    const float mrb1 = r.mrb1, mrb2 = r.mrb2, margin = r.margin, gap = r.gap;
     bool live = false;
     if (g1 >= 0 && (pid1 < 0 || pid1 < s.nprops) && (pid2 < 0 || pid2 < s.nprops)) {
       const float inc = detect ? margin : margin - gap;
@@ -82,6 +93,11 @@
         live = v3dot(df, df) <= r * r;
       }
     }
+    keep_live(mrb1); keep_live(mrb2); keep_live(margin); keep_live(gap); keep_live(b1); keep_live(b2); keep_live(type1);
+#pragma unroll
+    for (int k = 0; k < 3; k++) { keep_live(lp1[k]); keep_live(lp2[k]); }
+#pragma unroll
+    for (int k = 0; k < 4; k++) keep_live(lq1[k]);
     const unsigned long long m = __ballot(live);
     if (live) list[nsurv + __popcll(m & lt)] = (uint8_t)pr;
     nsurv += __popcll(m);
@@ -102,14 +118,15 @@
     int n = 0;
     FaceCand rc;
     unsigned rm = 0u;
+    const auto* R = &M->pair_rec[pr >= 0 ? pr : 0];
+    const int rec_single = R->single;
+    const float margin = R->margin, gap = R->gap;
     if (pr >= 0) {
-      const auto* R = &M->pair_rec[pr];
       const int b1 = R->b1, b2 = R->b2, pid1 = R->pid1, pid2 = R->pid2, type1 = R->type1;
       const float lp1[3] = {R->pos1[0], R->pos1[1], R->pos1[2]}, lp2[3] = {R->pos2[0], R->pos2[1], R->pos2[2]};
       const float lq1[4] = {R->quat1[0], R->quat1[1], R->quat1[2], R->quat1[3]};
       const float lq2[4] = {R->quat2[0], R->quat2[1], R->quat2[2], R->quat2[3]};
       const float ms1[3] = {R->size1[0], R->size1[1], R->size1[2]}, ms2[3] = {R->size2[0], R->size2[1], R->size2[2]};
-      const float margin = R->margin, gap = R->gap;
       float p1[3], R1[9], s1[3], p2[3], R2[9], s2[3], tmp[3], q[4];
       m3mulv(tmp, s.xmat[b1], lp1); v3add(p1, s.xpos[b1], tmp);
       qmul(q, s.xquat[b1], lq1); q2mat(R1, q);
@@ -119,7 +136,7 @@
       if (pid2 >= 0) v3copy(s2, s.prop_size[pid2]); else v3copy(s2, ms2);
       const float inc = detect ? margin : margin - gap;
       MRE_DBG_STAMP(6, 1);
-      if ((R->single >> 8) == 2) n = cyl_box(p1, R1, s1, p2, R2, s2[0], s2[2], inc, normal, buf);
+      if ((rec_single >> 8) == 2) n = cyl_box(p1, R1, s1, p2, R2, s2[0], s2[2], inc, normal, buf);
       else if (type1 == 0) n = plane_box(p1, R1, p2, R2, s2, inc, normal, buf);
       else n = box_box(p1, R1, s1, p2, R2, s2, inc, normal, buf, clip_always, rc, rm);
       MRE_DBG_STAMP(6, 2);
@@ -152,7 +169,8 @@
       }
     }
 #endif
-    const bool single = pr >= 0 && n > 1 && (M->pair_rec[pr].single & 0xFF) != 0;
+    keep_live(rec_single); keep_live(margin); keep_live(gap);
+    const bool single = pr >= 0 && n > 1 && (rec_single & 0xFF) != 0;
     const int ncand = n;
     if (single) n = 1;
     int off = base, tot = base;
@@ -166,7 +184,7 @@
       if (tot > NCON_MAX) s.overflow = 1;
     }
     if (single) {
-      const float incw = M->pair_rec[pr].margin - M->pair_rec[pr].gap;
+      const float incw = margin - gap;
       if (rm & FACE_IN_REGS) {
         float wsum = 0.f, px = 0.f, py = 0.f, pz = 0.f, dmin = 0.f, bx = 0.f, by = 0.f, bz = 0.f;
         bool first = true;
@@ -257,16 +275,17 @@
   return dmin + y * (dmax - dmin);
 }
 
-MRE_DEV void jac_robot(ModelP M, Sm& s, int rs, int b, const float* p, const float* ax, float sg) {
+MRE_DEV void jac_robot(Sm& s, int rs, const uint32_t* ch, const float* p, const float* ax, float sg, bool first) {
   float off[3];
   v3sub(off, p, s.com_robot);
-  const int n = M->chain_len[b];
-  for (int k = 0; k < n; k++) {
-    const int j = M->chain_dof[b][k];
-    const float* c = s.cdof[j];
-    float t[3];
-    v3cross(t, c, off);
-    s.Jr[rs][j] += sg * (ax[0] * (c[3] + t[0]) + ax[1] * (c[4] + t[1]) + ax[2] * (c[5] + t[2]));
+  const int n = jp_chain_len(ch);
+  uint64_t bits = jp_chain_bits(ch);
+  for (int k = 0; k < n; k++, bits >>= 4) {
+    const int j = (int)(bits & 15u);
+    const float term = jp_term(s.cdof[j], off, ax, sg);
+    float e = 0.f;
+    if (!first) e = s.Jr[rs][j];
+    s.Jr[rs][j] = jp_accumulate(e, term, first);
   }
 }
 MRE_DEV int row_blk(const Sm& s, int i, int& r) {
@@ -433,6 +452,11 @@
     const float lim_range[2] = {M->body_rec[limb].jnt_range[0], M->body_rec[limb].jnt_range[1]};
     const float opt_timestep = M->opt_rec.timestep, opt_impratio = M->opt_rec.impratio;
     const int opt_cone = M->opt_rec.cone;
+    const bool con_row = i >= 7 + nl;
+    const int cb1 = con_row ? (int)s.con_b1[(i - 7 - nl) / 3] : 0, cb2 = con_row ? (int)s.con_b2[(i - 7 - nl) / 3] : 0;
+    const auto* C1 = &M->chain_rec[cb1 < NRB ? cb1 : 0];
+    const auto* C2 = &M->chain_rec[cb2 < NRB ? cb2 : 0];
+    const uint32_t ch1[3] = {C1->w[0], C1->w[1], C1->w[2]}, ch2[3] = {C2->w[0], C2->w[1], C2->w[2]};
     if (i < 7) {
       rs = i;
       const int e = eqi;
@@ -497,7 +521,7 @@
       diag = invw1;
     } else {
       const int c = (i - 7 - nl) / 3, r = (i - 7 - nl) % 3;
-      const int b1 = s.con_b1[c], b2 = s.con_b2[c];
+      const int b1 = cb1, b2 = cb2;
       const float* ax = &s.con_frame[c][3 * r];
       const float* p = s.con_pos[c];
       const int rs0 = s.con_rslot[c];
@@ -505,11 +529,11 @@
       int slot = 0;
       float dg = 0.f;
       if (b1 > 0) {
-        if (b1 < NRB) { jac_robot(M, s, rs, b1, p, ax, -1.f); dg += invw1; }
+        if (b1 < NRB) { jac_robot(s, rs, ch1, p, ax, -1.f, true); dg += invw1; }
         else { pa = b1 - NRB; jac_prop(s, i, slot++, b1, p, ax, -1.f); dg += 1.0f / s.prop_mass[pa]; }
       }
       if (b2 > 0) {
-        if (b2 < NRB) { jac_robot(M, s, rs, b2, p, ax, 1.f); dg += invw2; }
+        if (b2 < NRB) { jac_robot(s, rs, ch2, p, ax, 1.f, !(b1 > 0 && b1 < NRB)); dg += invw2; }
         else {
           const int pid = b2 - NRB;
           if (slot == 0) pa = pid; else pb = pid;
@@ -534,6 +558,8 @@
     }
     keep_live(lim_range[0]); keep_live(lim_range[1]); keep_live(invw1); keep_live(invw2); keep_live(rec_friction);
     keep_live(rec_margin); keep_live(rec_gap); keep_live(opt_impratio); keep_live(opt_cone);
+#pragma unroll
+    for (int c = 0; c < 3; c++) { keep_live((int)ch1[c]); keep_live((int)ch2[c]); }
     s.hdr[i] = rs | (pa << 8) | (pb << 12);
     const float imp = impedance(solimp, imp_pos, margin);
     float tc = solref[0];
diff --git a/mujoco_robot_environments_amd/lib.py b/mujoco_robot_environments_amd/lib.py
--- a/mujoco_robot_environments_amd/lib.py
+++ b/mujoco_robot_environments_amd/lib.py
@@ -9,7 +9,7 @@
 _CSRC = os.path.join(os.path.dirname(os.path.abspath(__file__)), "csrc")
 _SO = os.path.join(_CSRC, "libmre.so")
 _SOURCES = ["mre_kernels.hip", "mre_render.hip", "mre_api.cpp"]
-_HEADERS = ["mre_dev.h", "mre_math.h", "mre_collide.h", "mre_solver.h", "mre_newton.h", "mre_osc.h",
+_HEADERS = ["mre_dev.h", "mre_math.h", "mre_collide.h", "mre_solver.h", "mre_newton.h", "mre_osc.h", "mre_jac_point.h",
             os.path.join("..", "..", "include", "mre.h")]
 _UNHASHED_SOURCES = ["mre_records.hip", "mre_records.h", "mre_labels.hip", "mre_labels.h", "mre_heightmap.hip", "mre_heightmap.h",
                      "mre_heightmap_point.h", "mre_warp.hip", "mre_warp.h", "mre_warp_point.h", "mre_model.cpp", "mre_model.h", "mre_sched.cpp", "mre_env.h",
```

New measurement: 24.93 million. 0.989x the previous value.
